# nlaha/genomics-rs

Measured on NVIDIA B200. Metric: GCUPS (affine NW/SW, score+traceback), higher is better.
Workload: dtype int32

## Files before the change

### genomics_rs_b200/_lib.py

```python
from __future__ import annotations

import ctypes as C
import os
import threading

_HERE = os.path.dirname(os.path.abspath(__file__))
LIB_PATH = os.environ.get("GX_LIB_PATH") or os.path.join(_HERE, "libgxalign.so")

GX_OK = 0
GX_FLAG_TRACEBACK = 1
GX_FLAG_LCS_AT_MAX = 2
GX_FLAG_START_CELL = 4

EXPORTS = [
    "gx_init", "gx_shutdown", "gx_device_count", "gx_strerror", "gx_last_error", "gx_version", "gx_check_scores",
    "gx_align_pair", "gx_align_batch", "gx_score_batch", "gx_plan_create", "gx_plan_upload", "gx_plan_execute",
    "gx_plan_fetch", "gx_plan_fetch_scores", "gx_plan_destroy", "gx_plan_stat", "gx_plan_debug_timeline", "gx_replay_ops", "gx_k0_measure",
    "gx_band_range", "gx_band_create", "gx_band_export", "gx_band_connect", "gx_band_upload", "gx_band_execute",
    "gx_band_score", "gx_band_stat", "gx_band_destroy", "gx_nw_score_banded", "gx_debug_planes", "gx_debug_tile_order",
]


class GxScores(C.Structure):
    _fields_ = [("s_match", C.c_int32), ("s_mismatch", C.c_int32), ("g", C.c_int32), ("h", C.c_int32)]


class GxResult(C.Structure):
    _fields_ = [
        ("score", C.c_int64),
        ("start_i", C.c_uint64), ("start_j", C.c_uint64), ("end_i", C.c_uint64), ("end_j", C.c_uint64),
        ("n_ops", C.c_uint64), ("matches", C.c_uint64), ("mismatches", C.c_uint64),
        ("gap_extensions", C.c_uint64), ("opening_gaps", C.c_uint64), ("lcs_at_first_max", C.c_uint64),
        ("fill_ms", C.c_double), ("walk_ms", C.c_double),
    ]


class GxError(RuntimeError):
    def __init__(self, status: int, detail: str = ""):
        self.status = status
        super().__init__(f"libgxalign status {status}: {detail}")


_lib = None
_lock = threading.Lock()
_inited_device = None


def load() -> C.CDLL:
    global _lib
    if _lib is not None:
        return _lib
    with _lock:
        if _lib is not None:
            return _lib
        if not os.path.exists(LIB_PATH):
            raise ImportError(
                f"{LIB_PATH} is missing: build it with `python -m genomics_rs_b200.build` "
                "(nvcc, sm_100a).  genomics_rs_b200 has no CPU or PyTorch fallback.")
        lib = C.CDLL(LIB_PATH)
        vp, u64, i32 = C.c_void_p, C.c_uint64, C.c_int
        lib.gx_init.argtypes = [i32]; lib.gx_init.restype = i32
        lib.gx_shutdown.argtypes = []; lib.gx_shutdown.restype = None
        lib.gx_device_count.argtypes = []; lib.gx_device_count.restype = i32
        lib.gx_strerror.argtypes = [i32]; lib.gx_strerror.restype = C.c_char_p
        lib.gx_last_error.argtypes = []; lib.gx_last_error.restype = C.c_char_p
        lib.gx_version.argtypes = []; lib.gx_version.restype = C.c_char_p
        lib.gx_check_scores.argtypes = [GxScores, u64, u64]; lib.gx_check_scores.restype = i32
        lib.gx_align_pair.argtypes = [vp, u64, vp, u64, GxScores, i32, i32, C.POINTER(GxResult), vp, u64]
        lib.gx_align_pair.restype = i32
        lib.gx_align_batch.argtypes = [vp, u64, vp, vp, vp, vp, u64, GxScores, i32, i32, vp, vp, vp]
        lib.gx_align_batch.restype = i32
        lib.gx_score_batch.argtypes = [vp, u64, vp, vp, vp, vp, u64, GxScores, i32, vp]
        lib.gx_score_batch.restype = i32
        lib.gx_plan_create.argtypes = [vp, vp, u64, GxScores, i32, i32, C.POINTER(vp)]; lib.gx_plan_create.restype = i32
        lib.gx_plan_upload.argtypes = [vp, vp, u64, vp, vp]; lib.gx_plan_upload.restype = i32
        lib.gx_plan_execute.argtypes = [vp]; lib.gx_plan_execute.restype = i32
        lib.gx_plan_fetch.argtypes = [vp, vp, vp, vp]; lib.gx_plan_fetch.restype = i32
        lib.gx_plan_fetch_scores.argtypes = [vp, vp]; lib.gx_plan_fetch_scores.restype = i32
        lib.gx_plan_destroy.argtypes = [vp]; lib.gx_plan_destroy.restype = None
        lib.gx_plan_stat.argtypes = [vp, i32]; lib.gx_plan_stat.restype = C.c_double
        lib.gx_plan_debug_timeline.argtypes = [vp, vp, u64]; lib.gx_plan_debug_timeline.restype = i32
        lib.gx_replay_ops.argtypes = [vp, u64, u64, u64, vp, vp]; lib.gx_replay_ops.restype = i32
        lib.gx_k0_measure.argtypes = [vp, i32]; lib.gx_k0_measure.restype = i32
        lib.gx_band_range.argtypes = [u64, i32, i32, C.POINTER(u64), C.POINTER(u64)]; lib.gx_band_range.restype = i32
        lib.gx_band_create.argtypes = [u64, u64, i32, i32, i32, GxScores, C.POINTER(vp)]; lib.gx_band_create.restype = i32
        lib.gx_band_export.argtypes = [vp, vp, u64]; lib.gx_band_export.restype = i32
        lib.gx_band_connect.argtypes = [vp, vp, vp]; lib.gx_band_connect.restype = i32
        lib.gx_band_upload.argtypes = [vp, vp, vp]; lib.gx_band_upload.restype = i32
        lib.gx_band_execute.argtypes = [vp]; lib.gx_band_execute.restype = i32
        lib.gx_band_score.argtypes = [vp, C.POINTER(C.c_int64), C.POINTER(i32)]; lib.gx_band_score.restype = i32
        lib.gx_band_stat.argtypes = [vp, i32]; lib.gx_band_stat.restype = C.c_double
        lib.gx_band_destroy.argtypes = [vp]; lib.gx_band_destroy.restype = None
        lib.gx_nw_score_banded.argtypes = [vp, u64, vp, u64, GxScores, i32, C.POINTER(C.c_int64)]
        lib.gx_nw_score_banded.restype = i32
        lib.gx_debug_tile_order.argtypes = [vp, vp, u64, i32, i32, vp, u64, C.POINTER(u64)]; lib.gx_debug_tile_order.restype = i32
        lib.gx_debug_planes.argtypes = [vp, u64, vp, u64, GxScores, i32, vp, vp, vp]; lib.gx_debug_planes.restype = i32
        _lib = lib
    return _lib


def check(status: int) -> None:
    if status != GX_OK:
        lib = load()
        detail = lib.gx_strerror(status).decode()
        extra = lib.gx_last_error().decode()
        raise GxError(status, f"{detail}{' -- ' + extra if extra else ''}")


def ensure_init(device: int | None = None) -> C.CDLL:
    global _inited_device
    lib = load()
    if _inited_device is None:
        if device is None:
            device = int(os.environ.get("LOCAL_RANK", "0"))
        check(lib.gx_init(device))
        _inited_device = device
    return lib


def shutdown() -> None:
    global _inited_device
    if _lib is not None and _inited_device is not None:
        _lib.gx_shutdown()
        _inited_device = None
```

### genomics_rs_b200/csrc/gx_api.cu

```cuda
#include <algorithm>
#include <cstdio>
#include <cstdlib>
#include <cstring>
#include <mutex>
#include <new>
#include <string>
#include <thread>
#include <vector>

#include "../../include/gxalign.h"
#include "gx_fill.cuh"
#include "gx_lcs.cuh"
#include "gx_reads.cuh"
#include "gx_walk.cuh"

namespace gx {

static_assert(sizeof(DevResult) == sizeof(gx_result), "DevResult must mirror gx_result");
static_assert(sizeof(PairDesc) == 104, "PairDesc layout");
static_assert(warp_smem_bytes(2) % 16 == 0 && warp_smem_bytes(4) % 16 == 0 && warp_smem_bytes(8) % 16 == 0 && warp_smem_bytes(16) % 16 == 0,
              "per-warp smem must keep 16 B alignment");

struct Block {
    void *ptr;
    size_t size;
    bool free;
};

struct Ctx {
    int device = -1;
    int sm_count = 0;
    cudaStream_t stream = nullptr;
    cudaEvent_t ev[4] = {nullptr, nullptr, nullptr, nullptr};
    std::vector<Block> pool;
    static constexpr int NLANES = 3;
    cudaStream_t lane_stream[NLANES] = {nullptr, nullptr, nullptr};
    cudaEvent_t lane_done[NLANES] = {nullptr, nullptr, nullptr};
    int *lane_scores_host[NLANES] = {nullptr, nullptr, nullptr};
    uint4 *lane_rec_host[NLANES] = {nullptr, nullptr, nullptr};
    size_t lane_scores_cap = 0;
    int host_threads = 1;
    uint8_t *ops_stage = nullptr;
    size_t ops_stage_cap = 0;
    std::string last_error;
    size_t pool_bytes = 0;
};

static Ctx *g_ctx = nullptr;
static std::recursive_mutex g_mu;
static thread_local std::string g_err;

static int fail_cuda(cudaError_t e, const char *what) {
    char buf[512];
    snprintf(buf, sizeof buf, "%s: %s (%s)", what, cudaGetErrorString(e), cudaGetErrorName(e));
    g_err = buf;
    if (g_ctx) g_ctx->last_error = buf;
    return GX_ERR_CUDA;
}
#define GX_GUARD_END                                                  \
    catch (const std::bad_alloc &) {                                  \
        g_err = "host allocation failed";                             \
        return GX_ERR_NOMEM;                                          \
    }                                                                 \
    catch (...) {                                                     \
        g_err = "unexpected C++ exception inside libgxalign";         \
        return GX_ERR_INTERNAL;                                       \
    }
#define CK(call)                                        \
    do {                                                \
        cudaError_t e__ = (call);                       \
        if (e__ != cudaSuccess) return fail_cuda(e__, #call); \
    } while (0)

static int pool_alloc(Ctx *c, size_t bytes, void **out) {
    if (bytes == 0) bytes = 16;
    bytes = (bytes + 511) & ~size_t(511);
    int best = -1;
    for (size_t k = 0; k < c->pool.size(); ++k) {
        Block &b = c->pool[k];
        if (b.free && b.size >= bytes && b.size <= 2 * bytes + (1u << 20))
            if (best < 0 || b.size < c->pool[best].size) best = (int)k;
    }
    if (best >= 0) {
        c->pool[best].free = false;
        *out = c->pool[best].ptr;
        return GX_OK;
    }
    void *p = nullptr;
    cudaError_t e = cudaMalloc(&p, bytes);
    if (e != cudaSuccess) {
        for (auto it = c->pool.begin(); it != c->pool.end();) {
            if (it->free) {
                cudaFree(it->ptr);
                c->pool_bytes -= it->size;
                it = c->pool.erase(it);
            } else ++it;
        }
        cudaGetLastError();
        e = cudaMalloc(&p, bytes);
        if (e != cudaSuccess) {
            cudaGetLastError();
            g_err = "device allocation of " + std::to_string(bytes) + " bytes failed";
            return GX_ERR_NOMEM;
        }
    }
    c->pool.push_back({p, bytes, false});
    c->pool_bytes += bytes;
    *out = p;
    return GX_OK;
}
static void pool_free(Ctx *c, void *p) {
    if (!p) return;
    for (auto &b : c->pool)
        if (b.ptr == p) {
            b.free = true;
            return;
        }
}

struct Tunables {
    int r = -1, batch = -1, code_band = -1, band_resident = 1;
    int k = -1, chain1 = -1, tickets = -1, resident = -1, wpc = -1, grid_cap = -1, pad_keys = 0, poll_nap = 0, start_lead = 0,
        fill_stats = 0, walk_stats = 0, walk_rows = 0, no_stream = 0, reads32 = 0, test_abort = 0;
};
static int env_int(const char *name, int dflt) {
    const char *e = getenv(name);
    return e ? atoi(e) : dflt;
}
static Tunables read_tunables() {
    Tunables t;
    t.k = env_int("GX_K", -1);
    t.r = env_int("GX_R", -1);
    t.batch = env_int("GX_BATCH", -1);
    t.band_resident = env_int("GX_BAND_RESIDENT", 1);
    t.code_band = env_int("GX_CODE_BAND", -1);
    t.chain1 = env_int("GX_CHAIN1", -1);
    t.tickets = getenv("GX_TICKETS") ? 1 : -1;
    t.resident = env_int("GX_RESIDENT", -1);
    t.wpc = env_int("GX_WPC", -1);
    t.grid_cap = env_int("GX_GRID_CAP", -1);
    t.pad_keys = getenv("GX_PAD_KEYS") ? 1 : 0;
    t.poll_nap = env_int("GX_POLL_NAP", 0);
    t.start_lead = env_int("GX_START_LEAD", 0);
    t.fill_stats = env_int("GX_FILL_STATS", 0);
    t.walk_stats = getenv("GX_WALK_STATS") ? 1 : 0;
    t.walk_rows = env_int("GX_WALK_ROWS", 0);
    t.no_stream = getenv("GX_NO_STREAM") ? 1 : 0;
    t.reads32 = getenv("GX_READS32") ? 1 : 0;
    t.test_abort = getenv("GX_TEST_ABORT") ? 1 : 0;
    return t;
}

enum PlanKind { KIND_WAVEFRONT = 0, KIND_READS = 1 };
typedef void (*FillKernel)(const FillParams);

}

struct gx_band;
struct gx_plan {
    gx::Ctx *ctx = nullptr;
    int kind = gx::KIND_WAVEFRONT;
    uint64_t n_pairs = 0;
    gx_scores sc{};
    gx::Tunables tun;
    int is_local = 0, flags = 0;
    int K = 8, R = 1;
    uint32_t cpb = 1;
    bool chain1 = false;
    int track = 0;
    bool traceback = false;
    std::vector<gx::PairDesc> pairs;
    std::vector<uint64_t> len1, len2;
    uint64_t n_tiles = 0;
    uint64_t n_strips = 0;
    uint64_t cells = 0;
    uint64_t code_bytes = 0, ops_bytes = 0, colbuf_entries = 0, top_entries = 0, progress_entries = 0, best_entries = 0;
    uint64_t blob_cap = 0;
    uint64_t max_len = 0;
    uint8_t *d_blob = nullptr;
    uint8_t *d_blob_sym = nullptr;
    uint8_t *d_lut = nullptr;
    unsigned long long *d_stats = nullptr;
    unsigned long long h_stats[8] = {0};
    unsigned long long *d_timeline = nullptr;
    bool prof = false;
    gx::PairDesc *d_pairs = nullptr;
    gx::TileDesc *d_tiles = nullptr;
    gx::TileDesc *d_strips = nullptr;
    bool resident = false;
    uint32_t pmax = 0;
    uint32_t *d_ctrl = nullptr;
    unsigned long long *d_colbuf = nullptr;
    int2 *d_top = nullptr;
    uint8_t *d_codes = nullptr;
    int4 *d_best = nullptr;
    bool lcs = false;
    int4 *d_first = nullptr;
    uint32_t *d_masks = nullptr, *d_carry = nullptr;
    uint32_t carry_words = 0;
    float lcs_ms = 0;
    gx::DevResult *d_results = nullptr;
    uint8_t *d_ops = nullptr;
    uint64_t *d_off1 = nullptr, *d_off2 = nullptr;
    uint32_t *d_len1 = nullptr, *d_len2 = nullptr;
    int *d_scores = nullptr;
    uint32_t parity = 0;
    bool uploaded = false, executed = false, colbuf_dirty = true;
    float fill_ms = 0, walk_ms = 0;
    int launches = 0;
    int retries = 0;
    int reads_bits = 0;
    bool code_band = false;
    uint8_t *d_tile_codes = nullptr;
    int band_fallbacks = 0;
    uint32_t left_band = 0;
    double code_cell_frac = 1.0;
    uint64_t h2d_bytes = 0, d2h_bytes = 0, dev_bytes = 0;
    gx_band *band = nullptr;
};

struct gx_band {
    gx_plan *plan = nullptr;
    uint64_t m = 0, n_total = 0;
    gx_scores sc{};
    int n_bands = 0, first = 0, last = 0;
    std::vector<uint64_t> col0, width;
    uint8_t *link = nullptr;
    std::vector<unsigned long long *> internal;
    void *left_base = nullptr, *right_base = nullptr;
    uint32_t epoch = 0;
    bool connected = false, poisoned = false, trivial = false;
    float fill_ms = 0;
};

namespace gx {

#define GX_COMBOS(X) X(4, 1) X(8, 1) X(16, 1)

#define GX_DECL(K, R)                                                  \
    FillKernel pick_fill_##K##_##R##_0(bool prof, bool L, bool C, int track); \
    FillKernel pick_fill_##K##_##R##_1(bool prof, bool L, bool C, int track);
GX_COMBOS(GX_DECL)
#undef GX_DECL

static bool combo_ok(int K, int R) {
#define GX_CHK(k, r) if (K == k && R == r) return true;
    GX_COMBOS(GX_CHK)
#undef GX_CHK
    return false;
}

static FillKernel pick_fill(int K, int R, bool prof, bool chain1, bool L, bool C, int track) {
#define GX_PICK(k, r) if (K == k && R == r) return chain1 ? pick_fill_##k##_##r##_1(prof, L, C, track) : pick_fill_##k##_##r##_0(prof, L, C, track);
    GX_COMBOS(GX_PICK)
#undef GX_PICK
    return nullptr;
}

static int launch_fill(gx_plan *pl, const FillParams &fp, int grid_cap, int track_override = -1) {
    Ctx *c = pl->ctx;
    const int K = pl->K;
    const bool L = pl->is_local != 0, C = pl->traceback;
    const bool banded = pl->code_band && track_override < 0 && C && !L;
    FillKernel kern = (track_override >= 0) ? pick_fill(K, pl->R, pl->prof, pl->chain1, L, false, track_override)
                      : banded              ? pick_fill(K, pl->R, pl->prof, pl->chain1, false, true, 4)
                                            : pick_fill(K, pl->R, pl->prof, pl->chain1, L, C, pl->track);
    if (!kern) {
        g_err = "no fill kernel for this (K, R)";
        return GX_ERR_INTERNAL;
    }
    int wpc = (pl->n_strips * 2 >= (uint64_t)c->sm_count * warps_per_sm(K)) ? WARPS_PER_CTA : 1;
    if (pl->tun.wpc >= 0) wpc = pl->tun.wpc == 1 ? 1 : WARPS_PER_CTA;
    if (pl->resident) wpc = 1;
    const size_t smem = (size_t)wpc * warp_smem_bytes(K);
    CK(cudaFuncSetAttribute(kern, cudaFuncAttributeMaxDynamicSharedMemorySize, (int)(WARPS_PER_CTA * warp_smem_bytes(K))));
    int occ = 0;
    CK(cudaOccupancyMaxActiveBlocksPerMultiprocessor(&occ, kern, wpc * 32, smem));
    if (occ < 1) occ = 1;
    const bool codes_kernel = C && track_override < 0;
    occ = std::min(occ, (codes_kernel ? warps_per_sm(K) : GX_SCORE_CTAS * WARPS_PER_CTA) / wpc);
    uint64_t cap = (uint64_t)c->sm_count * occ;
    FillParams fq = fp;
    fq.tile_codes = banded ? pl->d_tile_codes : nullptr;
    if (pl->resident && pl->n_strips > cap) {
        g_err = "resident-strips plan does not fit the device (fewer than 16 single-warp CTAs per SM)";
        return GX_ERR_INTERNAL;
    }
    if (pl->resident) {
        fq.pmax = pl->pmax;
        fq.tiles = pl->d_strips;
        fq.n_tiles = (uint32_t)(pl->n_strips * pl->pmax);
    }
    uint64_t want = fq.pmax ? pl->n_strips : (pl->n_tiles + wpc - 1) / wpc;
    if (pl->tun.grid_cap >= 0) grid_cap = pl->tun.grid_cap;
    if (grid_cap > 0 && (uint64_t)grid_cap < cap) cap = grid_cap;
    int grid = (int)std::min<uint64_t>(want, cap);
    if (grid < 1) grid = 1;
    if (pl->resident) {
        void *kargs[] = {(void *)&fq};
        CK(cudaLaunchCooperativeKernel((const void *)kern, dim3((unsigned)grid), dim3((unsigned)(wpc * 32)), kargs, smem, c->stream));
    } else {
        kern<<<grid, wpc * 32, smem, c->stream>>>(fq);
    }
    CK(cudaGetLastError());
    return GX_OK;
}

typedef void (*WalkKernel)(const WalkParams);
static int launch_walk(gx_plan *pl, WalkParams wp) {
    WalkKernel kern = nullptr;
#define GX_WALK(k, r) \
    if (pl->K == k && pl->R == r) kern = gx_walk_kernel<k, r>;
    GX_COMBOS(GX_WALK)
#undef GX_WALK
    if (!kern) {
        g_err = "no walk kernel for this (K, R)";
        return GX_ERR_INTERNAL;
    }
    const uint32_t row_cap = (uint32_t)std::max<uint64_t>(64, std::min<uint64_t>(512, (pl->max_len + 63) / 64 * 64));
    uint32_t rows = 0;
    for (uint32_t cand : {512u, 384u, 256u, 192u, 128u, 64u}) {
        if (cand > 256u && pl->K > 8) continue;
        const uint32_t r_ = std::min(cand, row_cap);
        const uint32_t per_sm = std::min<uint32_t>(2048u / WALK_THREADS, (227u * 1024u) / (walk_smem_bytes(pl->K, pl->R, r_) + 1024u));
        if (pl->n_pairs <= (uint64_t)per_sm * (uint64_t)pl->ctx->sm_count) {
            rows = r_;
            break;
        }
    }
    if (!rows) rows = pl->max_len <= 256 ? 64u : 128u;
    if (pl->tun.walk_rows >= 64 && pl->tun.walk_rows <= 512 && pl->tun.walk_rows % 64 == 0) rows = (uint32_t)pl->tun.walk_rows;
    wp.win_rows = rows;
    const uint32_t smem = wp.traceback ? walk_smem_bytes(pl->K, pl->R, rows) : 0u;
    CK(cudaFuncSetAttribute(kern, cudaFuncAttributeMaxDynamicSharedMemorySize, (int)walk_smem_bytes(pl->K, pl->R, 512u)));
    kern<<<(unsigned)pl->n_pairs, wp.traceback ? WALK_THREADS : 32, smem, pl->ctx->stream>>>(wp);
    CK(cudaGetLastError());
    return GX_OK;
}

static int check_scores_impl(gx_scores sc, uint64_t m, uint64_t n, bool local) {
    if (!(sc.h <= 0 && sc.g < 0 && (long long)sc.h + sc.g < 0)) return GX_ERR_SCORES;
    long long mx = std::max({std::llabs((long long)sc.s_match), std::llabs((long long)sc.s_mismatch), std::llabs((long long)sc.g)});
    long long lim = 1ll << 29;
    if (m > (1ull << 28) || n > (1ull << 28)) return GX_ERR_RANGE;
    if ((long long)(m + n + 2) * mx + std::llabs((long long)sc.h) >= lim) return GX_ERR_RANGE;
    if (local) {
        long long vmax = (long long)std::min(m, n) * std::max<long long>(sc.s_match, 0);
        if (vmax >= (1ll << 26)) return GX_ERR_RANGE;
    }
    return GX_OK;
}

static void plan_release(gx_plan *pl) {
    Ctx *c = pl->ctx;
    void *ptrs[] = {pl->d_tile_codes, pl->d_blob, pl->d_blob_sym, pl->d_lut, pl->d_stats, pl->d_timeline, pl->d_pairs, pl->d_tiles, pl->d_strips, pl->d_ctrl, pl->d_colbuf, pl->d_top, pl->d_codes, pl->d_best, pl->d_first, pl->d_masks, pl->d_carry,
                    pl->d_results, pl->d_ops, pl->d_off1, pl->d_off2, pl->d_len1, pl->d_len2, pl->d_scores};
    for (void *p : ptrs) pool_free(c, p);
}

}

using namespace gx;

extern "C" {

const char *gx_version(void) {
#ifdef GX_CHECKED
    return "gxalign 0.2 (sm_100a, checked build: device-side bounds assertions)";
#else
    return "gxalign 0.2 (sm_100a)";
#endif
}

const char *gx_strerror(int s) {
    switch (s) {
        case GX_OK: return "ok";
        case GX_ERR_ARG: return "invalid argument";
        case GX_ERR_SCORES: return "scores violate h <= 0, g < 0, h+g < 0";
        case GX_ERR_RANGE: return "sequence lengths x scores exceed the int32 cell range";
        case GX_ERR_OPS_CAP: return "ops buffer too small";
        case GX_ERR_NO_DEVICE: return "no sm_100 CUDA device (there is no CPU path)";
        case GX_ERR_CUDA: return "CUDA error";
        case GX_ERR_NOMEM: return "out of memory";
        case GX_ERR_NOT_INIT: return "gx_init not called";
        case GX_ERR_UNSUPPORTED: return "unsupported flag or mode";
        case GX_ERR_INTERNAL: return "internal error";
        default: return "unknown status";
    }
}

const char *gx_last_error(void) { return g_err.c_str(); }

int gx_device_count(void) {
    int n = 0;
    if (cudaGetDeviceCount(&n) != cudaSuccess) {
        cudaGetLastError();
        return 0;
    }
    int ok = 0;
    for (int d = 0; d < n; ++d) {
        int major = 0;
        if (cudaDeviceGetAttribute(&major, cudaDevAttrComputeCapabilityMajor, d) == cudaSuccess && major == 10) ok++;
    }
    return ok;
}

int gx_init(int device) try {
    std::lock_guard<std::recursive_mutex> lk(g_mu);
    int n = 0;
    if (cudaGetDeviceCount(&n) != cudaSuccess || n == 0) {
        cudaGetLastError();
        g_err = "no CUDA device visible";
        return GX_ERR_NO_DEVICE;
    }
    if (device < 0) {
        if (cudaGetDevice(&device) != cudaSuccess) return GX_ERR_NO_DEVICE;
    }
    if (device >= n) return GX_ERR_ARG;
    int major = 0;
    CK(cudaDeviceGetAttribute(&major, cudaDevAttrComputeCapabilityMajor, device));
    if (major != 10) {
        g_err = "device is not compute capability 10.x; libgxalign carries sm_100a code only";
        return GX_ERR_NO_DEVICE;
    }
    if (g_ctx && g_ctx->device == device) return GX_OK;
    if (g_ctx) return GX_ERR_ARG;
    CK(cudaSetDevice(device));
    Ctx *c = new (std::nothrow) Ctx();
    if (!c) return GX_ERR_NOMEM;
    c->device = device;
    CK(cudaDeviceGetAttribute(&c->sm_count, cudaDevAttrMultiProcessorCount, device));
    CK(cudaStreamCreateWithFlags(&c->stream, cudaStreamNonBlocking));
    for (auto &e : c->ev) CK(cudaEventCreate(&e));
    for (int k = 0; k < Ctx::NLANES; ++k) {
        CK(cudaStreamCreateWithFlags(&c->lane_stream[k], cudaStreamNonBlocking));
        CK(cudaEventCreateWithFlags(&c->lane_done[k], cudaEventDisableTiming));
    }
    {
        int ndev = 1;
        cudaGetDeviceCount(&ndev);
        const unsigned hw = std::thread::hardware_concurrency();
        c->host_threads = (int)std::max(1u, std::min(8u, hw / (unsigned)std::max(1, ndev)));
        if (const char *e = getenv("GX_HOST_THREADS")) c->host_threads = std::max(1, atoi(e));
    }
    g_ctx = c;
    return GX_OK;
}
GX_GUARD_END

static void band_cache_drop();
static void plan_cache_drop();

void gx_shutdown(void) {
    std::lock_guard<std::recursive_mutex> lk(g_mu);
    if (!g_ctx) return;
    cudaSetDevice(g_ctx->device);
    cudaStreamSynchronize(g_ctx->stream);
    band_cache_drop();
    plan_cache_drop();
    for (auto &b : g_ctx->pool) cudaFree(b.ptr);
    for (auto &e : g_ctx->ev) cudaEventDestroy(e);
    for (int k = 0; k < Ctx::NLANES; ++k) {
        if (g_ctx->lane_stream[k]) cudaStreamDestroy(g_ctx->lane_stream[k]);
        if (g_ctx->lane_done[k]) cudaEventDestroy(g_ctx->lane_done[k]);
        if (g_ctx->lane_scores_host[k]) cudaFreeHost(g_ctx->lane_scores_host[k]);
        if (g_ctx->lane_rec_host[k]) cudaFreeHost(g_ctx->lane_rec_host[k]);
    }
    if (g_ctx->ops_stage) cudaFreeHost(g_ctx->ops_stage);
    cudaStreamDestroy(g_ctx->stream);
    delete g_ctx;
    g_ctx = nullptr;
}

int gx_check_scores(gx_scores sc, uint64_t m, uint64_t n) { return check_scores_impl(sc, m, n, true); }

int gx_replay_ops(const uint8_t *ops, uint64_t n_ops, uint64_t start_i, uint64_t start_j, uint32_t *ops_i, uint32_t *ops_j) {
    if ((!ops && n_ops) || !ops_i || !ops_j) return GX_ERR_ARG;
    uint64_t i = start_i, j = start_j;
    for (uint64_t k = 0; k < n_ops; ++k) {
        ops_i[k] = (uint32_t)i;
        ops_j[k] = (uint32_t)j;
        switch (ops[k]) {
            case GX_MATCH:
            case GX_MISMATCH:
                i = i ? i - 1 : 0;
                j = j ? j - 1 : 0;
                break;
            case GX_INSERT:
            case GX_OPEN_INSERT: j = j ? j - 1 : 0; break;
            case GX_DELETE:
            case GX_OPEN_DELETE: i = i ? i - 1 : 0; break;
            default: return GX_ERR_ARG;
        }
    }
    return GX_OK;
}

}


static void build_ticket_order(const std::vector<uint32_t> &S, const std::vector<uint32_t> &P, const std::vector<uint64_t> &sbase,
                               std::vector<TileDesc> &tiles) {
    const size_t n_pairs = S.size();
    constexpr uint64_t TS = PANEL_H / 64;
    uint64_t vmax = 0;
    std::vector<uint32_t> live;
    for (size_t q = 0; q < n_pairs; ++q)
        if (S[q] && P[q]) {
            vmax = std::max<uint64_t>(vmax, (uint64_t)(P[q] - 1) * TS + sbase[q] + S[q] - 1);
            live.push_back((uint32_t)q);
        }
    for (uint64_t v = 0; v <= vmax && !live.empty(); ++v) {
        size_t keep = 0;
        for (size_t li = 0; li < live.size(); ++li) {
            const uint32_t q = live[li];
            const uint64_t last = (uint64_t)(P[q] - 1) * TS + sbase[q] + S[q] - 1;
            if (v <= last) live[keep++] = q;
            if (v < sbase[q]) continue;
            const uint64_t sv = v - sbase[q];
            const uint64_t p_hi = std::min<uint64_t>(P[q] - 1, sv / TS);
            const uint64_t p_lo = (sv >= S[q]) ? (sv - S[q] + 1 + TS - 1) / TS : 0;
            for (uint64_t p2 = p_lo; p2 <= p_hi; ++p2) tiles.push_back({q, (uint32_t)p2, (uint32_t)(sv - TS * p2), 0});
        }
        live.resize(keep);
    }
}

static int plan_create_locked(const uint64_t *len1, const uint64_t *len2, uint64_t n_pairs, gx_scores sc, int is_local, int flags,
                              const uint64_t *band_col0, gx_plan **out) {
    if (!out) return GX_ERR_ARG;
    *out = nullptr;
    if (!g_ctx) return GX_ERR_NOT_INIT;
    if ((!len1 || !len2) && n_pairs) return GX_ERR_ARG;
    if (n_pairs >= (1ull << 31)) return GX_ERR_RANGE;
    Ctx *c = g_ctx;
    CK(cudaSetDevice(c->device));
    uint64_t max_len = 0;
    for (uint64_t q = 0; q < n_pairs; ++q) {
        int rc = check_scores_impl(sc, len1[q], len2[q], is_local != 0);
        if (rc) return rc;
        max_len = std::max({max_len, len1[q], len2[q]});
    }
    if (n_pairs == 0) {
        int rc = check_scores_impl(sc, 0, 0, is_local != 0);
        if (rc) return rc;
    }
    gx_plan *pl = new (std::nothrow) gx_plan();
    if (!pl) return GX_ERR_NOMEM;
    pl->ctx = c;
    pl->n_pairs = n_pairs;
    pl->sc = sc;
    pl->tun = read_tunables();
    pl->is_local = is_local ? 1 : 0;
    pl->flags = flags;
    pl->traceback = (flags & GX_FLAG_TRACEBACK) != 0;
    pl->track = is_local ? ((pl->traceback || (flags & GX_FLAG_START_CELL)) ? 2 : 1) : 0;
    pl->len1.assign(len1, len1 + n_pairs);
    pl->len2.assign(len2, len2 + n_pairs);
    pl->max_len = max_len;
    for (uint64_t q = 0; q < n_pairs; ++q) pl->cells += (len1[q] + 1) * (len2[q] + 1);

    pl->lcs = (flags & GX_FLAG_LCS_AT_MAX) != 0 && !band_col0;
    if (pl->lcs) {
        long long mx = std::max({std::llabs((long long)sc.s_match), std::llabs((long long)sc.s_mismatch), std::llabs((long long)sc.g)});
        if (n_pairs > 65536 || (long long)(2 * max_len + 2) * mx + std::llabs((long long)sc.h) >= (1ll << 26)) {
            delete pl;
            return n_pairs > 65536 ? GX_ERR_UNSUPPORTED : GX_ERR_RANGE;
        }
    }
    const bool reads = !pl->lcs && !band_col0 && !pl->traceback && pl->track != 2 && n_pairs >= 1024 && max_len <= (uint64_t)READS_MAX_LEN &&
                       (!is_local || sc.s_mismatch < 0);
    pl->kind = reads ? KIND_READS : KIND_WAVEFRONT;
    int rc = GX_OK;
    auto A = [&](size_t bytes, void **p) {
        if (rc == GX_OK) {
            rc = pool_alloc(c, bytes, p);
            if (rc == GX_OK) pl->dev_bytes += (bytes + 511) & ~size_t(511);
        }
    };
    if (pl->kind == KIND_READS) {
        A(n_pairs * 8, (void **)&pl->d_off1);
        A(n_pairs * 8, (void **)&pl->d_off2);
        A(n_pairs * 4, (void **)&pl->d_len1);
        A(n_pairs * 4, (void **)&pl->d_len2);
        A(n_pairs * 4, (void **)&pl->d_scores);
        if (rc == GX_OK) {
            std::vector<uint32_t> l1(n_pairs), l2(n_pairs);
            for (uint64_t q = 0; q < n_pairs; ++q) {
                l1[q] = (uint32_t)len1[q];
                l2[q] = (uint32_t)len2[q];
            }
            cudaError_t e = cudaMemcpyAsync(pl->d_len1, l1.data(), n_pairs * 4, cudaMemcpyHostToDevice, c->stream);
            if (e == cudaSuccess) e = cudaMemcpyAsync(pl->d_len2, l2.data(), n_pairs * 4, cudaMemcpyHostToDevice, c->stream);
            if (e == cudaSuccess) e = cudaStreamSynchronize(c->stream);
            if (e != cudaSuccess) rc = fail_cuda(e, "upload lengths");
        }
        if (rc != GX_OK) {
            plan_release(pl);
            delete pl;
            return rc;
        }
        *out = pl;
        return GX_OK;
    }

    {
        const uint64_t resident = (uint64_t)c->sm_count * warps_per_sm(16);
        uint64_t strips16 = 0, strips8 = 0;
        for (uint64_t q = 0; q < n_pairs; ++q)
            if (len1[q] && len2[q]) {
                strips16 += (len2[q] + 511) / 512;
                strips8 += (len2[q] + 255) / 256;
            }
        (void)strips16;
        pl->K = (strips8 * 10 >= resident * 12 || max_len < 2048) ? 8 : 4;
        if (combo_ok(pl->tun.k, 1)) pl->K = pl->tun.k;
        pl->R = 1;
        if (pl->tun.r > 0 && combo_ok(pl->K, pl->tun.r)) pl->R = pl->tun.r;
        {
            uint64_t strips = 0;
            for (uint64_t q = 0; q < n_pairs; ++q)
                if (len1[q] && len2[q]) strips += (len2[q] + 32 * pl->K - 1) / (32 * pl->K);
            pl->chain1 = strips * 4 < resident;
            pl->n_strips = strips;
        }
        if (pl->tun.chain1 >= 0) pl->chain1 = pl->tun.chain1 != 0;
        const int kb = pl->K == 16 ? 4 : pl->K == 8 ? 3 : 2;
        if (pl->track == 2 && pl->chain1 && -((long long)sc.h + sc.g) >= (1ll << (31 - kb))) pl->chain1 = false;
    }
    const int K = pl->K, R = pl->R, W = 32 * K;
    {
        const uint64_t ns = pl->n_strips;
        pl->resident = ns > 0 && ns * 10 <= (uint64_t)c->sm_count * warps_per_sm(K) * 7 && pl->tun.tickets < 0;
        if (pl->tun.resident >= 0 && ns <= (uint64_t)c->sm_count * warps_per_sm(K)) pl->resident = pl->tun.resident != 0;
    }
    const uint32_t SPC = 64u / (uint32_t)(R * K), CPB_MAX = std::max(1u, 32u / (SPC * (uint32_t)R));
    {
        uint32_t steps = 32u;
        if (pl->tun.batch > 0) steps = (uint32_t)pl->tun.batch;
        uint32_t cpb = std::max(1u, steps / SPC);
        while (cpb & (cpb - 1)) cpb &= cpb - 1;
        pl->cpb = std::min(cpb, CPB_MAX);
    }
    const uint32_t CPB = pl->cpb, BATCH = CPB * SPC;
    pl->pairs.resize(n_pairs);
    std::vector<TileDesc> tiles;
    std::vector<uint64_t> sbase(n_pairs, 0);
    uint64_t n_tiles_total = 0;
    uint64_t colbuf = 0, top = 0, codes = 0, ops = 0, progress = 0, best = 0;
    uint64_t strip_base = 0;
    for (uint64_t q = 0; q < n_pairs; ++q) {
        PairDesc &pd = pl->pairs[q];
        memset(&pd, 0, sizeof pd);
        const uint64_t m = len1[q], n = len2[q];
        pd.m = (uint32_t)m;
        pd.n = (uint32_t)n;
        const bool interior = m > 0 && n > 0;
        pd.S = interior ? (uint32_t)((n + W - 1) / W) : 0;
        pd.P = interior ? (uint32_t)((m + PANEL_H - 1) / PANEL_H) : 0;
        pd.colbuf_off = colbuf;
        pd.top_off = top;
        pd.codes_off = codes;
        pd.ops_off = ops;
        pd.progress_off = (uint32_t)progress;
        pd.tile_base = (uint32_t)best;
        const uint32_t rows_max = (uint32_t)std::min<uint64_t>(m, PANEL_H);
        pd.tile_code_bytes = interior ? tile_batches(rows_max, (uint32_t)R, BATCH) * CPB * 32 * 16 : 0;
        pd.col0 = band_col0 ? (uint32_t)band_col0[q] : 0u;
        if (interior) {
            colbuf += (uint64_t)(pd.S - 1) * m;
            top += n;
            progress += pd.S;
            if (progress >= (1ull << 32) || best + (uint64_t)pd.S * pd.P >= (1ull << 32)) {
                delete pl;
                return GX_ERR_RANGE;
            }
            best += (uint64_t)pd.S * pd.P;
            if (pl->traceback) codes += (uint64_t)pd.S * pd.P * pd.tile_code_bytes;
        }
        if (pl->traceback) ops += ((m + n + 1) + 31) & ~uint64_t(31);
        sbase[q] = strip_base;
        n_tiles_total += (uint64_t)pd.S * pd.P;
        if (band_col0) strip_base += pd.S;
    }
    if (n_tiles_total >= (1ull << 32) - 65536) {
        delete pl;
        return GX_ERR_RANGE;
    }
    if (!pl->resident) {
        std::vector<uint32_t> Sv(n_pairs), Pv(n_pairs);
        for (uint64_t q = 0; q < n_pairs; ++q) {
            Sv[q] = pl->pairs[q].S;
            Pv[q] = pl->pairs[q].P;
        }
        tiles.reserve(n_tiles_total);
        build_ticket_order(Sv, Pv, sbase, tiles);
    }
    pl->n_tiles = n_tiles_total;
    std::vector<TileDesc> strips;
    {
        if (pl->resident) {
            for (uint64_t q = 0; q < n_pairs; ++q) pl->pmax = std::max(pl->pmax, pl->pairs[q].P);
            for (uint64_t q = 0; q < n_pairs; ++q)
                for (uint32_t s2 = 0; s2 < pl->pairs[q].S; ++s2)
                    for (uint32_t p2 = 0; p2 < pl->pmax; ++p2)
                        strips.push_back(p2 < pl->pairs[q].P ? TileDesc{(uint32_t)q, p2, s2, 0u} : TileDesc{0xffffffffu, 0u, 0u, 0u});
        }
    }
    pl->code_bytes = codes;
    pl->ops_bytes = ops;
    pl->colbuf_entries = colbuf;
    pl->top_entries = top;
    pl->progress_entries = progress;
    pl->best_entries = best;

    A(n_pairs * sizeof(PairDesc), (void **)&pl->d_pairs);
    A(tiles.size() * sizeof(TileDesc), (void **)&pl->d_tiles);
    if (pl->resident) A(strips.size() * sizeof(TileDesc), (void **)&pl->d_strips);
    A((16 + progress) * 4, (void **)&pl->d_ctrl);
    A(colbuf * 8, (void **)&pl->d_colbuf);
    A(top * 8, (void **)&pl->d_top);
    if (pl->traceback) A(codes, (void **)&pl->d_codes);
    if (pl->is_local) A(best * 16, (void **)&pl->d_best);
    if (pl->lcs) {
        pl->carry_words = (uint32_t)((max_len + 31) / 32 + 1);
        A(best * 16 + 16, (void **)&pl->d_first);
        A((size_t)n_pairs * 256 * LCS_BLOCK_WORDS * 4, (void **)&pl->d_masks);
        A((size_t)n_pairs * 2 * pl->carry_words * 4 + 16, (void **)&pl->d_carry);
    }
    A(n_pairs * sizeof(DevResult), (void **)&pl->d_results);
    std::vector<uint8_t> tile_codes;
    if (pl->traceback && !is_local && !band_col0 && (!pl->resident || pl->tun.band_resident != 0) && pl->tun.code_band != 0 && best > 0) {
        tile_codes.assign(best, 1);
        double with = 0, all = 0;
        for (uint64_t q = 0; q < n_pairs; ++q) {
            const PairDesc &pd = pl->pairs[q];
            const uint64_t dmn = pd.m > pd.n ? pd.m - pd.n : pd.n - pd.m;
            const uint64_t cw = pl->tun.code_band > 0 ? (uint64_t)pl->tun.code_band : 1024 + dmn;
            for (uint32_t p2 = 0; p2 < pd.P; ++p2) {
                const double rows = (double)std::min<uint64_t>(PANEL_H, pd.m - (uint64_t)p2 * PANEL_H);
                for (uint32_t s2 = 0; s2 < pd.S; ++s2) {
                    const double cols = (double)std::min<uint64_t>((uint64_t)W, pd.n - (uint64_t)s2 * W);
                    const bool in = tile_in_code_band(pd.m, pd.n, p2, s2, (uint32_t)W, cw);
                    tile_codes[pd.tile_base + (uint64_t)p2 * pd.S + s2] = in ? 1 : 0;
                    all += rows * cols;
                    if (in) with += rows * cols;
                }
            }
        }
        pl->code_cell_frac = all > 0 ? with / all : 1.0;
        pl->code_band = pl->code_cell_frac < 0.9;
        if (!pl->code_band) pl->code_cell_frac = 1.0;
        if (pl->code_band) A(best, (void **)&pl->d_tile_codes);
    }
    if (pl->traceback) A(ops, (void **)&pl->d_ops);
    if (rc == GX_OK && pl->code_band) {
        cudaError_t e = cudaMemcpyAsync(pl->d_tile_codes, tile_codes.data(), best, cudaMemcpyHostToDevice, c->stream);
        if (e == cudaSuccess) e = cudaStreamSynchronize(c->stream);
        if (e != cudaSuccess) rc = fail_cuda(e, "upload tile code flags");
    }
    if (rc == GX_OK && (!tiles.empty() || !strips.empty())) {
        cudaError_t e = cudaSuccess;
        if (!tiles.empty()) e = cudaMemcpyAsync(pl->d_tiles, tiles.data(), tiles.size() * sizeof(TileDesc), cudaMemcpyHostToDevice, c->stream);
        if (e == cudaSuccess && pl->resident)
            e = cudaMemcpyAsync(pl->d_strips, strips.data(), strips.size() * sizeof(TileDesc), cudaMemcpyHostToDevice, c->stream);
        if (e == cudaSuccess) e = cudaStreamSynchronize(c->stream);
        if (e != cudaSuccess) rc = fail_cuda(e, "upload tiles");
    }
    if (rc != GX_OK) {
        plan_release(pl);
        delete pl;
        return rc;
    }
    *out = pl;
    return GX_OK;
}


template <class F>
static void host_parallel(int threads, uint64_t n, F &&f) {
    if (threads <= 1 || n < (1u << 15)) {
        f(0, (uint64_t)0, n);
        return;
    }
    std::vector<std::thread> th;
    th.reserve(threads - 1);
    const uint64_t per = (n + threads - 1) / threads;
    for (int t = 1; t < threads; ++t) {
        const uint64_t lo = std::min<uint64_t>(n, per * t), hi = std::min<uint64_t>(n, per * (t + 1));
        th.emplace_back([&f, t, lo, hi] { f(t, lo, hi); });
    }
    f(0, (uint64_t)0, std::min<uint64_t>(n, per));
    for (auto &t : th) t.join();
}

static int score_batch_streamed(const uint8_t *blob, uint64_t blob_len, const uint64_t *off1, const uint64_t *len1,
                                const uint64_t *off2, const uint64_t *len2, uint64_t n_pairs, gx_scores sc, int is_local,
                                int64_t *scores, bool force32) {
    std::lock_guard<std::recursive_mutex> lk(g_mu);
    if (!g_ctx) return GX_ERR_NOT_INIT;
    Ctx *c = g_ctx;
    if (n_pairs < (1u << 18) || (is_local && sc.s_mismatch >= 0)) return GX_ERR_UNSUPPORTED;
    int rc = check_scores_impl(sc, READS_MAX_LEN, READS_MAX_LEN, is_local != 0);
    if (rc) return rc;
    CK(cudaSetDevice(c->device));
    constexpr int NL = Ctx::NLANES;
    const uint64_t CH = 1u << 18;
    const int T = std::min(c->host_threads, 16);
    if (c->lane_scores_cap < CH) {
        for (int k = 0; k < NL; ++k) {
            if (c->lane_scores_host[k]) cudaFreeHost(c->lane_scores_host[k]);
            c->lane_scores_host[k] = nullptr;
            if (c->lane_rec_host[k]) cudaFreeHost(c->lane_rec_host[k]);
            c->lane_rec_host[k] = nullptr;
            if (cudaHostAlloc((void **)&c->lane_scores_host[k], CH * sizeof(int), cudaHostAllocDefault) != cudaSuccess ||
                cudaHostAlloc((void **)&c->lane_rec_host[k], CH * sizeof(uint4), cudaHostAllocDefault) != cudaSuccess) {
                cudaGetLastError();
                c->lane_scores_cap = 0;
                return GX_ERR_NOMEM;
            }
        }
        c->lane_scores_cap = CH;
    }
    struct Lane {
        uint8_t *blob = nullptr;
        size_t blob_cap = 0;
        uint4 *rec = nullptr;
        int *scores = nullptr;
        uint64_t first = 0, count = 0;
        bool busy = false;
    } lane[NL];
    auto release = [&]() {
        for (auto &L : lane) {
            void *ptrs[] = {L.blob, L.rec, L.scores};
            for (void *p : ptrs) pool_free(c, p);
        }
    };
    auto drain = [&](int k) -> int {
        Lane &L = lane[k];
        if (!L.busy) return GX_OK;
        cudaError_t e = cudaEventSynchronize(c->lane_done[k]);
        if (e != cudaSuccess) return fail_cuda(e, "cudaEventSynchronize(lane_done)");
        const int *src = c->lane_scores_host[k];
        int64_t *dst = scores + L.first;
        for (uint64_t q = 0; q < L.count; ++q) dst[q] = src[q];
        L.busy = false;
        return GX_OK;
    };
    for (int k = 0; k < NL && rc == GX_OK; ++k) {
        Lane &L = lane[k];
        rc = pool_alloc(c, CH * sizeof(uint4), (void **)&L.rec);
        if (!rc) rc = pool_alloc(c, CH * 4, (void **)&L.scores);
    }
    struct Part {
        uint64_t lo = UINT64_MAX, hi = 0, maxlen = 0, sum = 0, bad = 0;
    };
    std::vector<Part> parts((size_t)std::max(T, 1));
#define CKB(call)                                   \
    {                                               \
        cudaError_t e__ = (call);                   \
        if (e__ != cudaSuccess) {                   \
            rc = fail_cuda(e__, #call);             \
            break;                                  \
        }                                           \
    }
    for (uint64_t first = 0, ci = 0; first < n_pairs && rc == GX_OK; first += CH, ++ci) {
        const int k = (int)(ci % NL);
        Lane &L = lane[k];
        const uint64_t count = std::min<uint64_t>(CH, n_pairs - first);
        const uint64_t *o1 = off1 + first, *o2 = off2 + first, *l1 = len1 + first, *l2 = len2 + first;
        for (auto &p : parts) p = Part();
        host_parallel(T, count, [&](int tid, uint64_t a, uint64_t b) {
            Part p;
            for (uint64_t q = a; q < b; ++q) {
                const uint64_t a0 = o1[q], a1 = a0 + l1[q], b0 = o2[q], b1 = b0 + l2[q];
                p.bad |= (uint64_t)(a1 > blob_len) | (uint64_t)(b1 > blob_len) | (uint64_t)(a1 < a0) | (uint64_t)(b1 < b0);
                p.lo = std::min(p.lo, std::min(a0, b0));
                p.hi = std::max(p.hi, std::max(a1, b1));
                p.maxlen = std::max(p.maxlen, std::max(l1[q], l2[q]));
                p.sum += l1[q] + l2[q];
            }
            parts[(size_t)tid] = p;
        });
        uint64_t lo = UINT64_MAX, hi = 0, maxlen = 0, sum = 0, badbits = 0;
        for (const auto &p : parts) {
            lo = std::min(lo, p.lo);
            hi = std::max(hi, p.hi);
            maxlen = std::max(maxlen, p.maxlen);
            sum += p.sum;
            badbits |= p.bad;
        }
        if (badbits) {
            rc = GX_ERR_ARG;
            break;
        }
        if (maxlen > (uint64_t)READS_MAX_LEN || hi - lo > 4 * sum + (1u << 20) || hi - lo >= (1ull << 32)) {
            rc = GX_ERR_UNSUPPORTED;
            break;
        }
        rc = drain(k);
        if (rc) break;
        const uint64_t span = hi > lo ? hi - lo : 0;
        if (L.blob_cap < span + 64) {
            pool_free(c, L.blob);
            L.blob = nullptr;
            L.blob_cap = 0;
            rc = pool_alloc(c, span + span / 4 + 64, (void **)&L.blob);
            if (rc) break;
            L.blob_cap = span + span / 4 + 64;
        }
        cudaStream_t st = c->lane_stream[k];
        if (span) CKB(cudaMemcpyAsync(L.blob, blob + lo, span, cudaMemcpyHostToDevice, st));
        {
            uint4 *rec = c->lane_rec_host[k];
            host_parallel(T, count, [&](int, uint64_t a, uint64_t b) {
                for (uint64_t q = a; q < b; ++q)
                    rec[q] = make_uint4((uint32_t)(o1[q] - lo), (uint32_t)(o2[q] - lo), (uint32_t)l1[q], (uint32_t)l2[q]);
            });
        }
        CKB(cudaMemcpyAsync(L.rec, c->lane_rec_host[k], count * sizeof(uint4), cudaMemcpyHostToDevice, st));
        ReadsParams rp;
        rp.blob = L.blob;
        rp.off1 = rp.off2 = nullptr;
        rp.len1 = rp.len2 = nullptr;
        rp.rec = L.rec;
        rp.n_pairs = (uint32_t)count;
        rp.scores = L.scores;
        rp.results = nullptr;
        rp.a = sc.s_match;
        rp.b = sc.s_mismatch;
        rp.g = sc.g;
        rp.h = sc.h;
        rp.is_local = is_local ? 1 : 0;
        if (launch_reads(rp, (int)maxlen, c->sm_count, st, force32) != 0) {
            rc = GX_ERR_UNSUPPORTED;
            break;
        }
        CKB(cudaGetLastError());
        CKB(cudaMemcpyAsync(c->lane_scores_host[k], L.scores, count * 4, cudaMemcpyDeviceToHost, st));
        CKB(cudaEventRecord(c->lane_done[k], st));
        L.first = first;
        L.count = count;
        L.busy = true;
    }
#undef CKB
    for (int k = 0; k < NL && rc == GX_OK; ++k) rc = drain(k);
    if (rc != GX_OK) {
        for (int k = 0; k < NL; ++k) cudaStreamSynchronize(c->lane_stream[k]);
        cudaGetLastError();
    }
    release();
    return rc;
}

extern "C" {

int gx_plan_create(const uint64_t *len1, const uint64_t *len2, uint64_t n_pairs, gx_scores sc, int is_local, int flags,
                   gx_plan **out) try {
    std::lock_guard<std::recursive_mutex> lk(g_mu);
    return plan_create_locked(len1, len2, n_pairs, sc, is_local, flags, nullptr, out);
}
GX_GUARD_END

int gx_plan_upload(gx_plan *pl, const uint8_t *blob, uint64_t blob_len, const uint64_t *off1, const uint64_t *off2) try {
    std::lock_guard<std::recursive_mutex> lk(g_mu);
    if (!pl || (!blob && blob_len) || ((!off1 || !off2) && pl->n_pairs)) return GX_ERR_ARG;
    Ctx *c = pl->ctx;
    CK(cudaSetDevice(c->device));
    for (uint64_t q = 0; q < pl->n_pairs; ++q)
        if (off1[q] > blob_len || pl->len1[q] > blob_len - off1[q] || off2[q] > blob_len || pl->len2[q] > blob_len - off2[q])
            return GX_ERR_ARG;
    if (!pl->d_blob || pl->blob_cap < blob_len + 64) {
        pool_free(c, pl->d_blob);
        pl->d_blob = nullptr;
        int rc = pool_alloc(c, blob_len + 64, (void **)&pl->d_blob);
        if (rc) return rc;
        pl->blob_cap = blob_len + 64;
        pl->dev_bytes += blob_len + 64;
    }
    if (blob_len) CK(cudaMemcpyAsync(pl->d_blob, blob, blob_len, cudaMemcpyHostToDevice, c->stream));
    CK(cudaMemsetAsync(pl->d_blob + blob_len, 0, 64, c->stream));
    pl->h2d_bytes = blob_len;
    if (pl->kind == KIND_READS) {
        if (pl->n_pairs) {
            CK(cudaMemcpyAsync(pl->d_off1, off1, pl->n_pairs * 8, cudaMemcpyHostToDevice, c->stream));
            CK(cudaMemcpyAsync(pl->d_off2, off2, pl->n_pairs * 8, cudaMemcpyHostToDevice, c->stream));
            pl->h2d_bytes += pl->n_pairs * 16;
        }
    } else {
        bool seen[256] = {false};
        int nsym = 0;
        uint8_t lut[256];
        memset(lut, 255, sizeof lut);
        {
            std::vector<std::pair<uint64_t, uint64_t>> segs;
            segs.reserve(2 * pl->n_pairs);
            for (uint64_t q = 0; q < pl->n_pairs; ++q) {
                segs.push_back({off1[q], pl->len1[q]});
                segs.push_back({off2[q], pl->len2[q]});
            }
            std::sort(segs.begin(), segs.end());
            segs.erase(std::unique(segs.begin(), segs.end()), segs.end());
            uint64_t done_to = 0;
            for (size_t k = 0; k < segs.size() && nsym <= 4; ++k) {
                uint64_t lo = std::max(segs[k].first, done_to), hi = segs[k].first + segs[k].second;
                for (uint64_t x = lo; x < hi; ++x) {
                    const uint8_t ch = blob[x];
                    if (!seen[ch]) {
                        seen[ch] = true;
                        if (nsym < 4) lut[ch] = (uint8_t)(8 * nsym);
                        nsym++;
                    }
                }
                done_to = std::max(done_to, hi);
            }
        }
        {
            const long long hg = (long long)pl->sc.h + pl->sc.g;
            const long long v[4] = {pl->sc.s_match - hg, pl->sc.s_mismatch - hg, pl->sc.s_match, pl->sc.s_mismatch};
            bool fits = true;
            for (long long x : v) fits = fits && x >= -128 && x <= 127;
            pl->prof = nsym <= 4 && fits && pl->n_tiles > 0;
        }
        if (pl->prof) {
            for (int x = 0; x < 256; ++x)
                if (lut[x] == 255) lut[x] = 0;
            if (!pl->d_lut) {
                int rc = pool_alloc(c, 256, (void **)&pl->d_lut);
                if (rc) return rc;
            }
            pool_free(c, pl->d_blob_sym);
            pl->d_blob_sym = nullptr;
            int rc = pool_alloc(c, blob_len + 64, (void **)&pl->d_blob_sym);
            if (rc) return rc;
            pl->dev_bytes += blob_len + 64;
            CK(cudaMemcpyAsync(pl->d_lut, lut, 256, cudaMemcpyHostToDevice, c->stream));
            const int grid = (int)std::min<uint64_t>((blob_len + 64 + 255) / 256, (uint64_t)c->sm_count * 8);
            gx_encode_kernel<<<grid, 256, 0, c->stream>>>(pl->d_blob, pl->d_blob_sym, (size_t)blob_len + 64, pl->d_lut);
            CK(cudaGetLastError());
        }
        for (uint64_t q = 0; q < pl->n_pairs; ++q) {
            pl->pairs[q].s1_off = off1[q];
            pl->pairs[q].s2_off = off2[q];
        }
        if (pl->n_pairs) {
            CK(cudaMemcpyAsync(pl->d_pairs, pl->pairs.data(), pl->n_pairs * sizeof(PairDesc), cudaMemcpyHostToDevice, c->stream));
            pl->h2d_bytes += pl->n_pairs * sizeof(PairDesc);
        }
    }
    CK(cudaStreamSynchronize(c->stream));
    pl->uploaded = true;
    return GX_OK;
}
GX_GUARD_END

static int plan_execute_once(gx_plan *pl, bool *aborted);

static int plan_build_tickets(gx_plan *pl) {
    Ctx *c = pl->ctx;
    const size_t np = pl->pairs.size();
    std::vector<uint32_t> Sv(np), Pv(np);
    std::vector<uint64_t> sbase(np, 0);
    uint64_t base = 0;
    for (size_t q = 0; q < np; ++q) {
        Sv[q] = pl->pairs[q].S;
        Pv[q] = pl->pairs[q].P;
        sbase[q] = base;
        if (pl->band) base += Sv[q];
    }
    std::vector<TileDesc> tiles;
    tiles.reserve(pl->n_tiles);
    build_ticket_order(Sv, Pv, sbase, tiles);
    if (tiles.size() != pl->n_tiles) return GX_ERR_INTERNAL;
    if (tiles.empty()) return GX_OK;
    pool_free(c, pl->d_tiles);
    pl->d_tiles = nullptr;
    int rc = pool_alloc(c, tiles.size() * sizeof(TileDesc), (void **)&pl->d_tiles);
    if (rc) return rc;
    CK(cudaMemcpyAsync(pl->d_tiles, tiles.data(), tiles.size() * sizeof(TileDesc), cudaMemcpyHostToDevice, c->stream));
    CK(cudaStreamSynchronize(c->stream));
    return GX_OK;
}

int gx_plan_execute(gx_plan *pl) try {
    std::lock_guard<std::recursive_mutex> lk(g_mu);
    if (!pl) return GX_ERR_ARG;
    if (!pl->uploaded) return GX_ERR_ARG;
    bool aborted = false;
    int rc = plan_execute_once(pl, &aborted);
    if (rc == GX_ERR_INTERNAL && aborted && pl->resident && !(pl->band && pl->band->n_bands > pl->band->last - pl->band->first)) {
        pl->resident = false;
        pl->retries++;
        int rb = plan_build_tickets(pl);
        if (rb) return rb;
        pl->colbuf_dirty = true;
        rc = plan_execute_once(pl, &aborted);
    }
    if (rc == GX_OK && pl->code_band && pl->left_band != 0) {
        const float f0 = pl->fill_ms, w0 = pl->walk_ms;
        const int l0 = pl->launches;
        pl->code_band = false;
        pl->code_cell_frac = 1.0;
        pl->band_fallbacks++;
        rc = plan_execute_once(pl, &aborted);
        pl->fill_ms += f0;
        pl->walk_ms += w0;
        pl->launches += l0;
    }
    return rc;
}
GX_GUARD_END

static int plan_execute_once(gx_plan *pl, bool *aborted) {
    Ctx *c = pl->ctx;
    CK(cudaSetDevice(c->device));
    pl->launches = 0;
    pl->fill_ms = pl->walk_ms = 0;
    const gx_scores sc = pl->sc;
    if (pl->n_pairs == 0) {
        pl->executed = true;
        return GX_OK;
    }
    if (pl->kind == KIND_READS) {
        ReadsParams rp;
        rp.blob = pl->d_blob;
        rp.off1 = pl->d_off1;
        rp.off2 = pl->d_off2;
        rp.len1 = pl->d_len1;
        rp.len2 = pl->d_len2;
        rp.rec = nullptr;
        rp.n_pairs = (uint32_t)pl->n_pairs;
        rp.scores = pl->d_scores;
        rp.results = nullptr;
        rp.a = sc.s_match;
        rp.b = sc.s_mismatch;
        rp.g = sc.g;
        rp.h = sc.h;
        rp.is_local = pl->is_local;
        CK(cudaEventRecord(c->ev[0], c->stream));
        int rc = launch_reads(rp, (int)pl->max_len, c->sm_count, c->stream, pl->tun.reads32 != 0, &pl->reads_bits);
        if (rc == -1) return GX_ERR_UNSUPPORTED;
        CK(cudaGetLastError());
        CK(cudaEventRecord(c->ev[1], c->stream));
        CK(cudaStreamSynchronize(c->stream));
        CK(cudaEventElapsedTime(&pl->fill_ms, c->ev[0], c->ev[1]));
        pl->launches = 1;
        pl->executed = true;
        return GX_OK;
    }

    gx_band *bd = pl->band;
    if (bd && bd->poisoned) {
        g_err = "band plan is unusable after a failed execute (neighbouring bands are out of step): create it again";
        return GX_ERR_INTERNAL;
    }
    CK(cudaEventRecord(c->ev[0], c->stream));
    if (pl->colbuf_dirty) {
        if (pl->colbuf_entries) CK(cudaMemsetAsync(pl->d_colbuf, 0xff, pl->colbuf_entries * 8, c->stream));
        if (bd) {
            if (bd->epoch != 0 && bd->n_bands > bd->last - bd->first) {
                bd->poisoned = true;
                return GX_ERR_INTERNAL;
            }
            for (auto *lk : bd->internal) CK(cudaMemsetAsync(lk, 0xff, bd->m * 8, c->stream));
        }
        pl->parity = 0;
    }
    pl->colbuf_dirty = true;
    CK(cudaMemsetAsync(pl->d_ctrl, 0, (16 + pl->progress_entries) * 4, c->stream));
    FillParams fp;
    fp.blob = pl->d_blob;
    fp.blob_sym = pl->prof ? pl->d_blob_sym : nullptr;
    fp.one = 1u;
    fp.stats = nullptr;
    fp.timeline = nullptr;
    fp.pad_keys = (sc.s_mismatch >= 0 || pl->tun.pad_keys) ? 1u : 0u;
    fp.poll_nap = (uint32_t)pl->tun.poll_nap;
    fp.start_lead = (uint32_t)pl->tun.start_lead;
    if (pl->tun.fill_stats) {
        if (!pl->d_stats) {
            int rc = pool_alloc(c, 64, (void **)&pl->d_stats);
            if (rc) return rc;
        }
        CK(cudaMemsetAsync(pl->d_stats, 0, 64, c->stream));
        fp.stats = pl->d_stats;
        if (pl->tun.fill_stats >= 2) {
            if (!pl->d_timeline) {
                int rc = pool_alloc(c, (std::max<uint64_t>(pl->n_tiles, pl->n_strips * pl->pmax) + 1) * 32, (void **)&pl->d_timeline);
                if (rc) return rc;
            }
            fp.timeline = pl->d_timeline;
        }
    }
    fp.pairs = pl->d_pairs;
    fp.n_pairs = (uint32_t)pl->n_pairs;
    fp.code_bytes = pl->code_bytes;
    fp.tiles = pl->d_tiles;
    fp.n_tiles = (uint32_t)pl->n_tiles;
    fp.pmax = 0;
    fp.parity = pl->parity;
    fp.cpb = pl->cpb;
    fp.epoch = bd ? bd->epoch + 1 : 0;
    fp.ticket = pl->d_ctrl;
    fp.progress = pl->d_ctrl + 16;
    fp.colbuf = pl->d_colbuf;
    fp.top = pl->d_top;
    fp.codes = pl->d_codes;
    fp.tile_best = pl->d_best;
    fp.g = sc.g;
    fp.h = sc.h;
    fp.hg = sc.h + sc.g;
    fp.ap = sc.s_match - fp.hg;
    fp.bp = sc.s_mismatch - fp.hg;
    if (pl->n_tiles) {
        int rc = launch_fill(pl, fp, 0);
        if (rc) return rc;
        pl->launches++;
    }
    CK(cudaEventRecord(c->ev[1], c->stream));
    if (bd && bd->left_base) {
        gx_band_ack_kernel<<<1, 1, 0, c->stream>>>(reinterpret_cast<uint32_t *>(bd->left_base), bd->epoch + 1);
        CK(cudaGetLastError());
        pl->launches++;
    }
    WalkParams wp;
    wp.blob = pl->d_blob;
    wp.pairs = pl->d_pairs;
    wp.n_pairs = (uint32_t)pl->n_pairs;
    wp.top = pl->d_top;
    wp.codes = pl->d_codes;
    wp.tile_best = pl->d_best;
    wp.results = pl->d_results;
    wp.ops = pl->d_ops;
    wp.g = sc.g;
    wp.h = sc.h;
    wp.hg = fp.hg;
    wp.kcols_log2 = pl->K == 16 ? 4 : pl->K == 4 ? 2 : 3;
    wp.is_local = pl->is_local;
    wp.traceback = pl->traceback ? 1 : 0;
    wp.have_best = pl->track == 2 ? 1 : 0;
    wp.debug = pl->tun.walk_stats;
    wp.check = pl->d_ctrl + 2;
    wp.left_band = pl->d_ctrl + 3;
    wp.tile_codes = pl->code_band ? pl->d_tile_codes : nullptr;
    wp.code_bytes = pl->code_bytes;
    wp.ops_bytes = pl->ops_bytes;
    {
        int rc = launch_walk(pl, wp);
        if (rc) return rc;
        pl->launches++;
    }
    CK(cudaEventRecord(c->ev[2], c->stream));
    uint32_t ctrl_words[3] = {0, 0, 0};
    CK(cudaMemcpyAsync(ctrl_words, pl->d_ctrl + 1, 12, cudaMemcpyDeviceToHost, c->stream));
    uint32_t ctrl2[2] = {0, 0};
    if (pl->lcs) {
        if (pl->n_tiles) {
            CK(cudaMemsetAsync(pl->d_ctrl, 0, (16 + pl->progress_entries) * 4, c->stream));
            FillParams fq = fp;
            fq.parity = pl->parity ^ 1u;
            fq.codes = nullptr;
            fq.tile_best = pl->d_first;
            fq.stats = nullptr;
            fq.timeline = nullptr;
            int rc = launch_fill(pl, fq, 0, 3);
            if (rc) return rc;
            pl->launches++;
            CK(cudaMemcpyAsync(ctrl2, pl->d_ctrl + 1, 8, cudaMemcpyDeviceToHost, c->stream));
        }
        LcsParams lp;
        lp.blob = pl->d_blob;
        lp.pairs = pl->d_pairs;
        lp.n_pairs = (uint32_t)pl->n_pairs;
        lp.tile_first = pl->d_first;
        lp.masks = pl->d_masks;
        lp.carry = pl->d_carry;
        lp.carry_words = pl->carry_words;
        lp.results = pl->d_results;
        gx_lcs_kernel<<<(unsigned)pl->n_pairs, 32, 0, c->stream>>>(lp);
        CK(cudaGetLastError());
        pl->launches++;
        CK(cudaEventRecord(c->ev[3], c->stream));
    }
    if (fp.stats) CK(cudaMemcpyAsync(pl->h_stats, pl->d_stats, 64, cudaMemcpyDeviceToHost, c->stream));
    CK(cudaStreamSynchronize(c->stream));
    uint32_t abort_word = ctrl_words[0];
    const uint32_t abort_word2 = ctrl2[0];
    if (ctrl_words[1] || ctrl2[1]) {
        g_err = "checked build: device bounds check failed at site " + std::to_string(ctrl_words[1] ? ctrl_words[1] : ctrl2[1]);
        return GX_ERR_INTERNAL;
    }
    if (pl->tun.test_abort && pl->resident && pl->retries == 0) abort_word = 1;
    if (abort_word || abort_word2) {
        g_err = "fill kernel aborted: a tile waited > SPIN_LIMIT polls for a dependency";
        if (bd && bd->n_bands > bd->last - bd->first) bd->poisoned = true;
        *aborted = true;
        return GX_ERR_INTERNAL;
    }
    if (bd) bd->epoch++;
    pl->left_band = ctrl_words[2];
    CK(cudaEventElapsedTime(&pl->fill_ms, c->ev[0], c->ev[1]));
    CK(cudaEventElapsedTime(&pl->walk_ms, c->ev[1], c->ev[2]));
    if (pl->lcs) CK(cudaEventElapsedTime(&pl->lcs_ms, c->ev[2], c->ev[3]));
    if (!(pl->lcs && pl->n_tiles)) pl->parity ^= 1u;
    pl->colbuf_dirty = false;
    pl->executed = true;
    return GX_OK;
}

int gx_plan_fetch(gx_plan *pl, gx_result *out, uint8_t *ops_blob, const uint64_t *ops_off) try {
    std::lock_guard<std::recursive_mutex> lk(g_mu);
    if (!pl || (!out && pl->n_pairs)) return GX_ERR_ARG;
    if (!pl->executed) return GX_ERR_ARG;
    if (pl->traceback && pl->n_pairs && (!ops_blob || !ops_off)) return GX_ERR_ARG;
    Ctx *c = pl->ctx;
    CK(cudaSetDevice(c->device));
    if (pl->n_pairs == 0) return GX_OK;
    if (pl->kind == KIND_READS) {
        std::vector<int> sc32(pl->n_pairs);
        CK(cudaMemcpyAsync(sc32.data(), pl->d_scores, pl->n_pairs * 4, cudaMemcpyDeviceToHost, c->stream));
        CK(cudaStreamSynchronize(c->stream));
        pl->d2h_bytes = pl->n_pairs * 4;
        for (uint64_t q = 0; q < pl->n_pairs; ++q) {
            gx_result r;
            memset(&r, 0, sizeof r);
            r.score = sc32[q];
            r.start_i = r.end_i = pl->len1[q];
            r.start_j = r.end_j = pl->len2[q];
            r.fill_ms = pl->fill_ms;
            out[q] = r;
        }
        return GX_OK;
    }
    CK(cudaMemcpyAsync(out, pl->d_results, pl->n_pairs * sizeof(gx_result), cudaMemcpyDeviceToHost, c->stream));
    pl->d2h_bytes = pl->n_pairs * sizeof(gx_result);
    if (pl->traceback) {
        if (c->ops_stage_cap < pl->ops_bytes) {
            if (c->ops_stage) cudaFreeHost(c->ops_stage);
            c->ops_stage = nullptr;
            c->ops_stage_cap = 0;
            const size_t want = pl->ops_bytes + pl->ops_bytes / 4 + 4096;
            if (cudaHostAlloc((void **)&c->ops_stage, want, cudaHostAllocDefault) != cudaSuccess) {
                cudaGetLastError();
                return GX_ERR_NOMEM;
            }
            c->ops_stage_cap = want;
        }
        CK(cudaMemcpyAsync(c->ops_stage, pl->d_ops, pl->ops_bytes, cudaMemcpyDeviceToHost, c->stream));
        pl->d2h_bytes += pl->ops_bytes;
    }
    CK(cudaStreamSynchronize(c->stream));
    int rc = GX_OK;
    const bool walk_dbg = pl->tun.walk_stats != 0;
    for (uint64_t q = 0; q < pl->n_pairs; ++q) {
        if (!walk_dbg) out[q].fill_ms = pl->fill_ms;
        if (!walk_dbg) out[q].walk_ms = pl->walk_ms;
        if (pl->traceback) {
            const uint64_t cap = ops_off[q + 1] - ops_off[q];
            if (out[q].n_ops > cap) {
                rc = GX_ERR_OPS_CAP;
                continue;
            }
            memcpy(ops_blob + ops_off[q], c->ops_stage + pl->pairs[q].ops_off, out[q].n_ops);
        }
    }
    return rc;
}
GX_GUARD_END

int gx_plan_fetch_scores(gx_plan *pl, int64_t *scores) try {
    std::lock_guard<std::recursive_mutex> lk(g_mu);
    if (!pl || (!scores && pl->n_pairs)) return GX_ERR_ARG;
    if (!pl->executed) return GX_ERR_ARG;
    Ctx *c = pl->ctx;
    CK(cudaSetDevice(c->device));
    if (pl->n_pairs == 0) return GX_OK;
    if (pl->kind == KIND_READS) {
        std::vector<int> sc32(pl->n_pairs);
        CK(cudaMemcpyAsync(sc32.data(), pl->d_scores, pl->n_pairs * 4, cudaMemcpyDeviceToHost, c->stream));
        CK(cudaStreamSynchronize(c->stream));
        pl->d2h_bytes = pl->n_pairs * 4;
        for (uint64_t q = 0; q < pl->n_pairs; ++q) scores[q] = sc32[q];
        return GX_OK;
    }
    std::vector<gx_result> res(pl->n_pairs);
    CK(cudaMemcpyAsync(res.data(), pl->d_results, pl->n_pairs * sizeof(gx_result), cudaMemcpyDeviceToHost, c->stream));
    CK(cudaStreamSynchronize(c->stream));
    pl->d2h_bytes = pl->n_pairs * sizeof(gx_result);
    for (uint64_t q = 0; q < pl->n_pairs; ++q) scores[q] = res[q].score;
    return GX_OK;
}
GX_GUARD_END

int gx_plan_debug_timeline(gx_plan *pl, uint64_t *out, uint64_t cap_words) {
    std::lock_guard<std::recursive_mutex> lk(g_mu);
    if (!pl || !out || !pl->d_timeline || cap_words < pl->n_tiles * 4) return GX_ERR_ARG;
    CK(cudaSetDevice(pl->ctx->device));
    CK(cudaMemcpy(out, pl->d_timeline, pl->n_tiles * 32, cudaMemcpyDeviceToHost));
    return GX_OK;
}

int gx_debug_tile_order(const uint64_t *len1, const uint64_t *len2, uint64_t n_pairs, int K, int bands, uint32_t *out,
                        uint64_t cap_tiles, uint64_t *n_tiles) try {
    if ((!len1 || !len2) && n_pairs) return GX_ERR_ARG;
    if (!n_tiles || (K != 2 && K != 4 && K != 8 && K != 16)) return GX_ERR_ARG;
    std::vector<uint32_t> S(n_pairs), P(n_pairs);
    std::vector<uint64_t> sbase(n_pairs, 0);
    uint64_t base = 0, total = 0;
    for (uint64_t q = 0; q < n_pairs; ++q) {
        const bool interior = len1[q] > 0 && len2[q] > 0;
        S[q] = interior ? (uint32_t)((len2[q] + 32 * K - 1) / (32 * K)) : 0;
        P[q] = interior ? (uint32_t)((len1[q] + PANEL_H - 1) / PANEL_H) : 0;
        sbase[q] = base;
        if (bands) base += S[q];
        total += (uint64_t)S[q] * P[q];
    }
    *n_tiles = total;
    if (!out) return GX_OK;
    if (cap_tiles < total) return GX_ERR_ARG;
    std::vector<TileDesc> tiles;
    tiles.reserve(total);
    build_ticket_order(S, P, sbase, tiles);
    if (tiles.size() != total) return GX_ERR_INTERNAL;
    for (size_t k = 0; k < tiles.size(); ++k) {
        out[3 * k + 0] = tiles[k].pair;
        out[3 * k + 1] = tiles[k].p;
        out[3 * k + 2] = tiles[k].s;
    }
    return GX_OK;
}
GX_GUARD_END

double gx_plan_stat(const gx_plan *pl, int what) {
    if (!pl) return -1.0;
    switch (what) {
        case 0: return pl->fill_ms;
        case 1: return pl->walk_ms;
        case 2: return pl->launches;
        case 3: return (double)pl->cells;
        case 4: return (double)pl->code_bytes;
        case 5: return (double)pl->dev_bytes;
        case 6: return (double)pl->h2d_bytes;
        case 7: return (double)pl->d2h_bytes;
        case 8: return (double)pl->n_tiles;
        case 9: return (double)pl->kind;
        case 15: return (double)pl->K;
        case 19: return (double)pl->R;
        case 20: return (double)pl->retries;
        case 23: return pl->code_cell_frac;
        case 24: return (double)pl->band_fallbacks;
        case 22: return (double)(pl->cpb * (64u / (uint32_t)(pl->R * pl->K)));
        case 21: return pl->resident ? 1.0 : 0.0;
        case 17: return pl->chain1 ? 1.0 : 0.0;
        case 18: return pl->lcs_ms;
        case 25: return pl->prof ? 1.0 : 0.0;
        case 26: return (double)pl->reads_bits;
        case 10: case 11: case 12: case 13: case 14: return (double)pl->h_stats[what - 10];
        default: return -1.0;
    }
}

void gx_plan_destroy(gx_plan *pl) {
    std::lock_guard<std::recursive_mutex> lk(g_mu);
    if (!pl) return;
    plan_release(pl);
    delete pl;
}


int gx_band_range(uint64_t n_total, int n_bands, int band, uint64_t *col0, uint64_t *width) {
    if (n_bands < 1 || band < 0 || band >= n_bands || !col0 || !width) return GX_ERR_ARG;
    uint64_t lo, hi;
    if (n_total / (uint64_t)n_bands >= std::max<uint64_t>(4096, 512ull * n_bands)) {
        const uint64_t base = ((n_total + n_bands - 1) / n_bands + 511) / 512 * 512;
        lo = std::min<uint64_t>(n_total, base * band);
        hi = std::min<uint64_t>(n_total, base * (band + 1));
    } else {
        const uint64_t q = n_total / n_bands, r = n_total % n_bands;
        lo = q * band + std::min<uint64_t>(band, r);
        hi = lo + q + ((uint64_t)band < r ? 1 : 0);
    }
    *col0 = lo;
    *width = hi - lo;
    return GX_OK;
}

static void band_free(gx_band *b) {
    if (!b) return;
    if (b->plan) gx_plan_destroy(b->plan);
    if (g_ctx) {
        for (auto *p : b->internal) pool_free(g_ctx, p);
        if (b->left_base) cudaIpcCloseMemHandle(b->left_base);
        if (b->right_base) cudaIpcCloseMemHandle(b->right_base);
        if (b->link) cudaFree(b->link);
        cudaGetLastError();
    }
    delete b;
}

int gx_band_create(uint64_t m, uint64_t n_total, int n_bands, int first_band, int last_band, gx_scores sc, gx_band **out) try {
    std::lock_guard<std::recursive_mutex> lk(g_mu);
    if (!out) return GX_ERR_ARG;
    *out = nullptr;
    if (!g_ctx) return GX_ERR_NOT_INIT;
    if (n_bands < 1 || first_band < 0 || last_band <= first_band || last_band > n_bands) return GX_ERR_ARG;
    int rc = check_scores_impl(sc, m, n_total, false);
    if (rc) return rc;
    if (m > 0 && n_total > 0 && n_total < (uint64_t)n_bands) return GX_ERR_ARG;
    Ctx *c = g_ctx;
    CK(cudaSetDevice(c->device));
    gx_band *b = new (std::nothrow) gx_band();
    if (!b) return GX_ERR_NOMEM;
    b->m = m;
    b->n_total = n_total;
    b->sc = sc;
    b->n_bands = n_bands;
    b->first = first_band;
    b->last = last_band;
    b->trivial = (m == 0 || n_total == 0);
    if (b->trivial) {
        *out = b;
        return GX_OK;
    }
    const int nl = last_band - first_band;
    std::vector<uint64_t> l1(nl, m), l2(nl);
    b->col0.resize(nl);
    b->width.resize(nl);
    for (int q = 0; q < nl; ++q) {
        gx_band_range(n_total, n_bands, first_band + q, &b->col0[q], &b->width[q]);
        l2[q] = b->width[q];
        if (l2[q] == 0) {
            delete b;
            return GX_ERR_ARG;
        }
    }
    rc = plan_create_locked(l1.data(), l2.data(), (uint64_t)nl, sc, 0, 0, b->col0.data(), &b->plan);
    if (rc) {
        delete b;
        return rc;
    }
    b->plan->band = b;
    for (int q = 0; q + 1 < nl && rc == GX_OK; ++q) {
        unsigned long long *p = nullptr;
        rc = pool_alloc(c, m * 8, (void **)&p);
        if (rc == GX_OK) b->internal.push_back(p);
    }
    if (rc == GX_OK && nl < n_bands) {
        cudaError_t e = cudaMalloc((void **)&b->link, 256 + m * 8);
        if (e == cudaSuccess) e = cudaMemsetAsync(b->link, 0xff, 256 + m * 8, c->stream);
        if (e == cudaSuccess) e = cudaMemsetAsync(b->link, 0, 256, c->stream);
        if (e == cudaSuccess) e = cudaStreamSynchronize(c->stream);
        if (e != cudaSuccess) {
            cudaGetLastError();
            rc = (e == cudaErrorMemoryAllocation) ? GX_ERR_NOMEM : fail_cuda(e, "band link block");
        }
    }
    if (rc != GX_OK) {
        band_free(b);
        return rc;
    }
    for (int q = 0; q < nl; ++q) {
        PairDesc &pd = b->plan->pairs[q];
        pd.inbox = (q > 0) ? b->internal[q - 1] : nullptr;
        pd.outbox = (q + 1 < nl) ? b->internal[q] : nullptr;
        pd.ack = nullptr;
    }
    b->connected = (nl == n_bands);
    *out = b;
    return GX_OK;
}
GX_GUARD_END

int gx_band_export(gx_band *b, void *handle, uint64_t handle_cap) {
    std::lock_guard<std::recursive_mutex> lk(g_mu);
    if (!b || !handle || handle_cap < GX_BAND_HANDLE_BYTES) return GX_ERR_ARG;
    static_assert(sizeof(cudaIpcMemHandle_t) <= GX_BAND_HANDLE_BYTES, "handle size");
    memset(handle, 0, GX_BAND_HANDLE_BYTES);
    if (!b->link) return GX_OK;
    CK(cudaSetDevice(g_ctx->device));
    cudaIpcMemHandle_t h;
    CK(cudaIpcGetMemHandle(&h, b->link));
    memcpy(handle, &h, sizeof h);
    return GX_OK;
}

int gx_band_connect(gx_band *b, const void *left_handle, const void *right_handle) try {
    std::lock_guard<std::recursive_mutex> lk(g_mu);
    if (!b) return GX_ERR_ARG;
    if (b->trivial) return GX_OK;
    const bool need_left = b->first > 0, need_right = b->last < b->n_bands;
    if ((need_left && !left_handle) || (need_right && !right_handle)) return GX_ERR_ARG;
    if (b->connected) return GX_OK;
    CK(cudaSetDevice(g_ctx->device));
    const int nl = b->last - b->first;
    if (need_left) {
        cudaIpcMemHandle_t h;
        memcpy(&h, left_handle, sizeof h);
        CK(cudaIpcOpenMemHandle(&b->left_base, h, cudaIpcMemLazyEnablePeerAccess));
        b->plan->pairs[0].inbox = reinterpret_cast<const unsigned long long *>(b->link + 256);
    }
    if (need_right) {
        cudaIpcMemHandle_t h;
        memcpy(&h, right_handle, sizeof h);
        CK(cudaIpcOpenMemHandle(&b->right_base, h, cudaIpcMemLazyEnablePeerAccess));
        b->plan->pairs[nl - 1].outbox = reinterpret_cast<unsigned long long *>(static_cast<uint8_t *>(b->right_base) + 256);
        b->plan->pairs[nl - 1].ack = reinterpret_cast<const uint32_t *>(b->link);
    }
    b->connected = true;
    if (b->plan->uploaded) {
        CK(cudaMemcpyAsync(b->plan->d_pairs, b->plan->pairs.data(), nl * sizeof(PairDesc), cudaMemcpyHostToDevice, g_ctx->stream));
        CK(cudaStreamSynchronize(g_ctx->stream));
    }
    return GX_OK;
}
GX_GUARD_END

int gx_band_upload(gx_band *b, const uint8_t *s1, const uint8_t *s2) try {
    std::lock_guard<std::recursive_mutex> lk(g_mu);
    if (!b) return GX_ERR_ARG;
    if (b->trivial) return GX_OK;
    if (!s1 || !s2) return GX_ERR_ARG;
    const int nl = b->last - b->first;
    const uint64_t c_lo = b->col0[0], c_hi = b->col0[nl - 1] + b->width[nl - 1];
    std::vector<uint8_t> blob(b->m + (c_hi - c_lo));
    memcpy(blob.data(), s1, b->m);
    memcpy(blob.data() + b->m, s2 + c_lo, c_hi - c_lo);
    std::vector<uint64_t> off1(nl, 0), off2(nl);
    for (int q = 0; q < nl; ++q) off2[q] = b->m + (b->col0[q] - c_lo);
    return gx_plan_upload(b->plan, blob.data(), blob.size(), off1.data(), off2.data());
}
GX_GUARD_END

int gx_band_execute(gx_band *b) try {
    std::lock_guard<std::recursive_mutex> lk(g_mu);
    if (!b) return GX_ERR_ARG;
    if (b->trivial) return GX_OK;
    if (!b->connected) return GX_ERR_ARG;
    int rc = gx_plan_execute(b->plan);
    b->fill_ms = b->plan->fill_ms;
    return rc;
}
GX_GUARD_END

int gx_band_score(gx_band *b, int64_t *score, int *valid) try {
    std::lock_guard<std::recursive_mutex> lk(g_mu);
    if (!b || !score || !valid) return GX_ERR_ARG;
    *valid = (b->last == b->n_bands) ? 1 : 0;
    *score = 0;
    if (!*valid) return GX_OK;
    if (b->trivial) {
        const uint64_t len = b->m + b->n_total;
        *score = len ? (int64_t)b->sc.h + (int64_t)len * b->sc.g : 0;
        return GX_OK;
    }
    if (!b->plan->executed) return GX_ERR_ARG;
    const int nl = b->last - b->first;
    std::vector<int64_t> sc(nl);
    int rc = gx_plan_fetch_scores(b->plan, sc.data());
    if (rc) return rc;
    *score = sc[nl - 1];
    return GX_OK;
}
GX_GUARD_END

double gx_band_stat(const gx_band *b, int what) {
    if (!b) return -1.0;
    if (what == 16) return (double)b->epoch;
    if (!b->plan) return what == 3 ? (double)((b->m + 1) * (b->n_total + 1)) : 0.0;
    return gx_plan_stat(b->plan, what);
}

void gx_band_destroy(gx_band *b) {
    std::lock_guard<std::recursive_mutex> lk(g_mu);
    band_free(b);
}

static gx_band *g_band_cache = nullptr;
static void band_cache_drop() {
    if (g_band_cache) band_free(g_band_cache);
    g_band_cache = nullptr;
}

int gx_nw_score_banded(const uint8_t *s1, uint64_t m, const uint8_t *s2, uint64_t n, gx_scores sc, int n_bands, int64_t *score) try {
    std::lock_guard<std::recursive_mutex> lk(g_mu);
    if (!score || (!s1 && m) || (!s2 && n)) return GX_ERR_ARG;
    gx_band *b = g_band_cache;
    const bool hit = b && b->m == m && b->n_total == n && b->n_bands == n_bands && b->first == 0 && b->last == n_bands &&
                     memcmp(&b->sc, &sc, sizeof sc) == 0 && !b->poisoned;
    if (!hit) {
        band_cache_drop();
        b = nullptr;
        int rc = gx_band_create(m, n, n_bands, 0, n_bands, sc, &b);
        if (rc) return rc;
        g_band_cache = b;
    }
    int valid = 0;
    int rc = gx_band_upload(b, s1, s2);
    if (!rc) rc = gx_band_execute(b);
    if (!rc) rc = gx_band_score(b, score, &valid);
    if (rc) band_cache_drop();
    return rc;
}
GX_GUARD_END

int gx_debug_planes(const uint8_t *s1, uint64_t m, const uint8_t *s2, uint64_t n, gx_scores sc, int is_local, int64_t *ins,
                    int64_t *del, int64_t *sub) try {
    std::lock_guard<std::recursive_mutex> lk(g_mu);
    if (!ins || !del || !sub || (!s1 && m) || (!s2 && n)) return GX_ERR_ARG;
    if (!g_ctx) return GX_ERR_NOT_INIT;
    if (!(m < 200 && n < 2000)) return GX_ERR_RANGE;
    int rc = check_scores_impl(sc, m, n, is_local != 0);
    if (rc) return rc;
    Ctx *c = g_ctx;
    CK(cudaSetDevice(c->device));
    const size_t cells = (size_t)(m + 1) * (n + 1);
    uint8_t *d_seq = nullptr;
    long long *d_planes = nullptr;
    rc = pool_alloc(c, m + n + 16, (void **)&d_seq);
    if (!rc) rc = pool_alloc(c, 3 * cells * 8, (void **)&d_planes);
    if (!rc) {
        cudaError_t e = cudaSuccess;
        if (m) e = cudaMemcpyAsync(d_seq, s1, m, cudaMemcpyHostToDevice, c->stream);
        if (e == cudaSuccess && n) e = cudaMemcpyAsync(d_seq + m, s2, n, cudaMemcpyHostToDevice, c->stream);
        if (e == cudaSuccess) {
            PlanesParams pp;
            pp.s1 = d_seq;
            pp.s2 = d_seq + m;
            pp.m = (uint32_t)m;
            pp.n = (uint32_t)n;
            pp.a = sc.s_match;
            pp.b = sc.s_mismatch;
            pp.g = sc.g;
            pp.h = sc.h;
            pp.is_local = is_local ? 1 : 0;
            pp.pi = d_planes;
            pp.pd = d_planes + cells;
            pp.ps = d_planes + 2 * cells;
            gx_planes_kernel<<<1, 256, 0, c->stream>>>(pp);
            e = cudaGetLastError();
        }
        if (e == cudaSuccess) e = cudaMemcpyAsync(ins, d_planes, cells * 8, cudaMemcpyDeviceToHost, c->stream);
        if (e == cudaSuccess) e = cudaMemcpyAsync(del, d_planes + cells, cells * 8, cudaMemcpyDeviceToHost, c->stream);
        if (e == cudaSuccess) e = cudaMemcpyAsync(sub, d_planes + 2 * cells, cells * 8, cudaMemcpyDeviceToHost, c->stream);
        if (e == cudaSuccess) e = cudaStreamSynchronize(c->stream);
        if (e != cudaSuccess) rc = fail_cuda(e, "gx_debug_planes");
    }
    pool_free(c, d_seq);
    pool_free(c, d_planes);
    return rc;
}
GX_GUARD_END

static gx_plan *g_plan_cache = nullptr;
static void plan_cache_drop() {
    if (g_plan_cache) gx_plan_destroy(g_plan_cache);
    g_plan_cache = nullptr;
}
static int cached_plan(const uint64_t *len1, const uint64_t *len2, uint64_t n_pairs, gx_scores sc, int is_local, int flags, gx_plan **out) {
    gx_plan *pl = g_plan_cache;
    const Tunables now = read_tunables();
    if (pl && pl->n_pairs == n_pairs && pl->is_local == (is_local ? 1 : 0) && pl->flags == flags && memcmp(&pl->sc, &sc, sizeof sc) == 0 &&
        memcmp(&pl->tun, &now, sizeof now) == 0 && (n_pairs == 0 || (len1 && len2 && memcmp(pl->len1.data(), len1, n_pairs * 8) == 0 &&
                                                                     memcmp(pl->len2.data(), len2, n_pairs * 8) == 0))) {
        *out = pl;
        return GX_OK;
    }
    plan_cache_drop();
    int rc = gx_plan_create(len1, len2, n_pairs, sc, is_local, flags, &pl);
    if (rc) return rc;
    g_plan_cache = pl;
    *out = pl;
    return GX_OK;
}

int gx_align_batch(const uint8_t *seq_blob, uint64_t blob_len, const uint64_t *off1, const uint64_t *len1, const uint64_t *off2,
                   const uint64_t *len2, uint64_t n_pairs, gx_scores sc, int is_local, int flags, gx_result *out,
                   uint8_t *ops_blob, const uint64_t *ops_off) try {
    std::lock_guard<std::recursive_mutex> lk(g_mu);
    gx_plan *pl = nullptr;
    int rc = cached_plan(len1, len2, n_pairs, sc, is_local, flags, &pl);
    if (rc) return rc;
    rc = gx_plan_upload(pl, seq_blob, blob_len, off1, off2);
    if (!rc) rc = gx_plan_execute(pl);
    if (!rc) rc = gx_plan_fetch(pl, out, ops_blob, ops_off);
    if (rc) plan_cache_drop();
    return rc;
}
GX_GUARD_END

int gx_score_batch(const uint8_t *seq_blob, uint64_t blob_len, const uint64_t *off1, const uint64_t *len1, const uint64_t *off2,
                   const uint64_t *len2, uint64_t n_pairs, gx_scores sc, int is_local, int64_t *scores) try {
    if ((!seq_blob && blob_len) || ((!off1 || !len1 || !off2 || !len2 || !scores) && n_pairs)) return GX_ERR_ARG;
    if (!getenv("GX_NO_STREAM")) {
        const int rcs = score_batch_streamed(seq_blob, blob_len, off1, len1, off2, len2, n_pairs, sc, is_local, scores,
                                             getenv("GX_READS32") != nullptr);
        if (rcs != GX_ERR_UNSUPPORTED) return rcs;
    }
    std::lock_guard<std::recursive_mutex> lk(g_mu);
    gx_plan *pl = nullptr;
    int rc = cached_plan(len1, len2, n_pairs, sc, is_local, 0, &pl);
    if (rc) return rc;
    rc = gx_plan_upload(pl, seq_blob, blob_len, off1, off2);
    if (!rc) rc = gx_plan_execute(pl);
    if (!rc) rc = gx_plan_fetch_scores(pl, scores);
    if (rc) plan_cache_drop();
    return rc;
}
GX_GUARD_END

int gx_align_pair(const uint8_t *s1, uint64_t m, const uint8_t *s2, uint64_t n, gx_scores sc, int is_local, int flags,
                  gx_result *out, uint8_t *ops, uint64_t ops_cap) try {
    if (!out || (!s1 && m) || (!s2 && n)) return GX_ERR_ARG;
    if (m > (1ull << 28) || n > (1ull << 28)) return GX_ERR_RANGE;
    if ((flags & GX_FLAG_TRACEBACK) && (!ops || ops_cap < m + n + 1)) return (!ops) ? GX_ERR_ARG : GX_ERR_OPS_CAP;
    std::vector<uint8_t> blob(m + n);
    if (m) memcpy(blob.data(), s1, m);
    if (n) memcpy(blob.data() + m, s2, n);
    uint64_t off1 = 0, off2 = m, l1 = m, l2 = n;
    uint64_t ops_off[2] = {0, ops_cap};
    return gx_align_batch(blob.data(), m + n, &off1, &l1, &off2, &l2, 1, sc, is_local, flags, out, ops, ops_off);
}
GX_GUARD_END

}
```

### genomics_rs_b200/csrc/gx_common.cuh

```cuda
#pragma once
#include <cuda_runtime.h>
#include <stdint.h>

namespace gx {

constexpr int NEG32 = -(1 << 30);

#ifndef GX_PANEL_LOG2
#define GX_PANEL_LOG2 12
#endif
constexpr int PANEL_H_LOG2 = GX_PANEL_LOG2;
constexpr int PANEL_H = 1 << PANEL_H_LOG2;
constexpr int WARPS_PER_CTA = 8;
constexpr int CTA_THREADS = WARPS_PER_CTA * 32;
__host__ __device__ constexpr int ctas_per_sm(int K) { return K > 0 ? 2 : 2; }
__host__ __device__ constexpr int warps_per_sm(int K) { return WARPS_PER_CTA * ctas_per_sm(K); }

constexpr int WARP_SMEM_S1 = PANEL_H + 32;
constexpr int WARP_SMEM_BYTES = WARP_SMEM_S1 + 512 + 512 + 16;
__host__ __device__ constexpr int warp_smem_bytes(int ) { return WARP_SMEM_BYTES; }

#ifdef GX_CHECKED
#define GX_CHECK(word, cond, site)                                   \
    do {                                                             \
        if (!(cond)) atomicMax(reinterpret_cast<unsigned int *>(word), (unsigned int)(site)); \
    } while (0)
#else
#define GX_CHECK(word, cond, site) ((void)0)
#endif

struct PairDesc {
    uint64_t s1_off, s2_off;
    uint64_t colbuf_off;
    uint64_t top_off;
    uint64_t codes_off;
    uint64_t ops_off;
    uint32_t m, n;
    uint32_t S, P;
    uint32_t progress_off;
    uint32_t tile_base;
    uint32_t tile_code_bytes;
    uint32_t col0;
    const unsigned long long *inbox;
    unsigned long long *outbox;
    const uint32_t *ack;
};

__host__ inline bool tile_in_code_band(uint64_t m, uint64_t n, uint32_t p, uint32_t s, uint32_t W, uint64_t code_w) {
    const uint64_t i0 = (uint64_t)p << PANEL_H_LOG2;
    const uint64_t i1 = (i0 + PANEL_H < m) ? i0 + PANEL_H : m;
    const uint64_t lo = i0 * n / m, hi = i1 * n / m;
    const uint64_t c0 = (uint64_t)s * W, c1 = c0 + W;
    return c1 + code_w > lo && c0 < hi + code_w + 1;
}

struct TileDesc {
    uint32_t pair, p, s, pad_;
};

struct DevResult {
    long long score;
    unsigned long long start_i, start_j, end_i, end_j, n_ops, matches, mismatches, gap_extensions, opening_gaps, lcs_at_first_max;
    double fill_ms, walk_ms;
};

struct FillParams {
    const uint8_t *blob;
    const uint8_t *blob_sym;
    uint32_t one;
    const PairDesc *pairs;
    const TileDesc *tiles;
    uint32_t n_pairs;
    uint32_t n_tiles;
    uint32_t pmax;
    uint32_t parity;
    uint32_t cpb;
    uint32_t epoch;
    uint32_t *ticket;
    uint32_t *progress;
    unsigned long long *colbuf;
    int2 *top;
    uint8_t *codes;
    const uint8_t *tile_codes;
    uint64_t code_bytes;
    int4 *tile_best;
    uint32_t pad_keys;
    uint32_t poll_nap;
    uint32_t start_lead;
    unsigned long long *timeline;
    unsigned long long *stats;
    int g, hg, ap, bp, h;
};

struct WalkParams {
    const uint8_t *blob;
    const PairDesc *pairs;
    uint32_t n_pairs;
    const int2 *top;
    const uint8_t *codes;
    const int4 *tile_best;
    DevResult *results;
    uint8_t *ops;
    int g, hg, h;
    int kcols_log2;
    int is_local, traceback, have_best;
    int debug;
    uint32_t *left_band;
    const uint8_t *tile_codes;
    uint32_t *check;
    uint64_t code_bytes, ops_bytes;
    uint32_t win_rows;
};

__device__ __forceinline__ uint32_t smem_u32(const void *p) { return (uint32_t)__cvta_generic_to_shared(p); }

__device__ __forceinline__ void mbar_init(uint64_t *bar, uint32_t count) {
    asm volatile("mbarrier.init.shared::cta.b64 [%0], %1;" ::"r"(smem_u32(bar)), "r"(count) : "memory");
}
__device__ __forceinline__ void mbar_expect_tx(uint64_t *bar, uint32_t bytes) {
    asm volatile("mbarrier.arrive.expect_tx.shared::cta.b64 _, [%0], %1;" ::"r"(smem_u32(bar)), "r"(bytes) : "memory");
}
__device__ __forceinline__ bool mbar_try_wait(uint64_t *bar, uint32_t phase) {
    uint32_t ok;
    asm volatile(
        "{\n\t.reg .pred p;\n\t"
        "mbarrier.try_wait.parity.shared::cta.b64 p, [%1], %2;\n\t"
        "selp.u32 %0, 1, 0, p;\n\t}"
        : "=r"(ok)
        : "r"(smem_u32(bar)), "r"(phase)
        : "memory");
    return ok != 0;
}
__device__ __forceinline__ void tma_bulk_g2s(void *dst_smem, const void *src_gmem, uint32_t bytes, uint64_t *bar) {
    asm volatile("cp.async.bulk.shared::cluster.global.mbarrier::complete_tx::bytes [%0], [%1], %2, [%3];" ::"r"(smem_u32(dst_smem)),
                 "l"(src_gmem), "r"(bytes), "r"(smem_u32(bar))
                 : "memory");
}
__device__ __forceinline__ void fence_proxy_async_smem() { asm volatile("fence.proxy.async.shared::cta;" ::: "memory"); }
__device__ __forceinline__ void fence_mbar_init() { asm volatile("fence.mbarrier_init.release.cluster;" ::: "memory"); }

__device__ __forceinline__ unsigned long long ld_relaxed_u64(const unsigned long long *p) {
    unsigned long long v;
    asm volatile("ld.relaxed.gpu.global.u64 %0, [%1];" : "=l"(v) : "l"(p) : "memory");
    return v;
}
__device__ __forceinline__ void st_relaxed_u64(unsigned long long *p, unsigned long long v) {
    asm volatile("st.relaxed.gpu.global.u64 [%0], %1;" ::"l"(p), "l"(v) : "memory");
}
__device__ __forceinline__ unsigned long long ld_relaxed_sys_u64(const unsigned long long *p) {
    unsigned long long v;
    asm volatile("ld.relaxed.sys.global.u64 %0, [%1];" : "=l"(v) : "l"(p) : "memory");
    return v;
}
__device__ __forceinline__ void st_relaxed_sys_u64(unsigned long long *p, unsigned long long v) {
    asm volatile("st.relaxed.sys.global.u64 [%0], %1;" ::"l"(p), "l"(v) : "memory");
}
__device__ __forceinline__ uint32_t ld_acquire_sys_u32(const uint32_t *p) {
    uint32_t v;
    asm volatile("ld.acquire.sys.global.u32 %0, [%1];" : "=r"(v) : "l"(p) : "memory");
    return v;
}
__device__ __forceinline__ void st_release_sys_u32(uint32_t *p, uint32_t v) {
    asm volatile("st.release.sys.global.u32 [%0], %1;" ::"l"(p), "r"(v) : "memory");
}
__device__ __forceinline__ uint32_t ld_relaxed_u32(const uint32_t *p) {
    uint32_t v;
    asm volatile("ld.relaxed.gpu.global.u32 %0, [%1];" : "=r"(v) : "l"(p) : "memory");
    return v;
}
__device__ __forceinline__ uint32_t ld_acquire_u32(const uint32_t *p) {
    uint32_t v;
    asm volatile("ld.acquire.gpu.global.u32 %0, [%1];" : "=r"(v) : "l"(p) : "memory");
    return v;
}
__device__ __forceinline__ void st_release_u32(uint32_t *p, uint32_t v) {
    asm volatile("st.release.gpu.global.u32 [%0], %1;" ::"l"(p), "r"(v) : "memory");
}
__device__ __forceinline__ int2 ld_cg_int2(const int2 *p) {
    int2 v;
    asm volatile("ld.global.cg.v2.s32 {%0,%1}, [%2];" : "=r"(v.x), "=r"(v.y) : "l"(p) : "memory");
    return v;
}
__device__ __forceinline__ void st_cg_int2(int2 *p, int2 v) {
    asm volatile("st.global.cg.v2.s32 [%0], {%1,%2};" ::"l"(p), "r"(v.x), "r"(v.y) : "memory");
}
__device__ __forceinline__ void st_cs_uint4(uint4 *p, uint4 v) {
    asm volatile("st.global.cs.v4.u32 [%0], {%1,%2,%3,%4};" ::"l"(p), "r"(v.x), "r"(v.y), "r"(v.z), "r"(v.w) : "memory");
}

__device__ __forceinline__ uint2 lds_volatile_uint2(const uint2 *p) {
    uint2 v;
    asm volatile("ld.volatile.shared.v2.u32 {%0,%1}, [%2];" : "=r"(v.x), "=r"(v.y) : "r"(smem_u32(p)) : "memory");
    return v;
}

__device__ __forceinline__ unsigned long long globaltimer_ns() {
    unsigned long long t;
    asm volatile("mov.u64 %0, %%globaltimer;" : "=l"(t));
    return t;
}

template <int N>
struct Log2 {
    static constexpr int value = 1 + Log2<N / 2>::value;
};
template <>
struct Log2<1> {
    static constexpr int value = 0;
};

}
```

### genomics_rs_b200/csrc/gx_fill.cuh

```cuda
#pragma once
#include <type_traits>

#include "gx_common.cuh"

namespace gx {

constexpr unsigned FULL = 0xffffffffu;
constexpr uint32_t SPIN_LIMIT = 1u << 22;

__device__ __forceinline__ bool spin_check(uint32_t &spins, uint32_t *abort_word) {
    if (++spins > SPIN_LIMIT) atomicExch(abort_word, 1u);
    if ((spins & 63u) == 0u || spins > SPIN_LIMIT) {
        if (*reinterpret_cast<volatile uint32_t *>(abort_word) != 0u) return true;
    }
    return false;
}

template <int N, class F>
__device__ __forceinline__ void static_for(F &&f) {
    if constexpr (N > 0) {
        static_for<N - 1>(f);
        f(std::integral_constant<int, N - 1>{});
    }
}

template <uint32_t UNIT>
__device__ __forceinline__ void code_acc(uint32_t &cw, int S, int I, int V, uint32_t one) {
    asm("{\n\t.reg .pred p1, p2;\n\t"
        "setp.ne.s32 p1, %1, %3;\n\t"
        "setp.ne.and.s32 p2, %2, %3, p1;\n\t"
        "@p1 mad.lo.u32 %0, %4, %5, %0;\n\t"
        "@p2 mad.lo.u32 %0, %4, %5, %0;\n\t}"
        : "+r"(cw)
        : "r"(S), "r"(I), "r"(V), "r"(one), "n"(UNIT));
}

#ifndef GX_SCORE_CTAS
#define GX_SCORE_CTAS 2
#endif
template <int K, int R>
struct Geo {
    static_assert(R * K <= 64 && (R & (R - 1)) == 0 && (K & (K - 1)) == 0, "R x K cells must fit one 16-byte code chunk");
    static constexpr int W = 32 * K;
    static constexpr int SPC = 64 / (R * K);
    static constexpr int CPB_MAX = 32 / (SPC * R) > 0 ? 32 / (SPC * R) : 1;
    static constexpr int KB = Log2<K>::value;
    static_assert(SPC * R <= 32, "one chunk must not exceed 32 rows");
};
__host__ __device__ __forceinline__ uint32_t tile_batches(uint32_t rows, uint32_t R, uint32_t batch) {
    return ((rows + R - 1) / R + 31 + batch - 1) / batch;
}

__device__ __forceinline__ void lds_over_if(int &x, int &y, const uint2 *p, bool pred) {
    asm volatile("{\n\t.reg .pred q;\n\tsetp.ne.u32 q, %3, 0;\n\t@q ld.shared.v2.u32 {%0,%1}, [%2];\n\t}"
                 : "+r"(x), "+r"(y)
                 : "r"(smem_u32(p)), "r"((uint32_t)pred));
}

template <int K, int R, bool LOCAL, bool CODES, int TRACK, bool PROF, bool MASKED, bool PAD, bool CHAIN1, bool THRU = false>
__device__ __forceinline__ void run_batch(int (&eu)[K], int (&du)[K], const int (&c2)[K], int (&eo)[R], int (&io)[R], int &vd,
                                          int &best, int &best_r, const int g, const int hg, const int ap, const int bp,
                                          const uint32_t one, const uint8_t *s1base ,
                                          const int (&prof4)[K] ,
                                          const uint2 *inr , uint2 *outring, uint4 *code_dst,
                                          const int t0, const int rows, const int lane, const int kvalid,
                                          int (&c1a)[R] , const int cpb ,
                                          uint32_t *chk , const int s1lo, const int s1hi ) {
    using G = Geo<K, R>;
    constexpr int KB = G::KB;
    const bool lane0 = lane == 0;
    auto s1char = [&](int r) __attribute__((always_inline)) -> int {
        if (MASKED) return (int)s1base[min(max(r, 0), rows - 1)];
        GX_CHECK(chk, r >= s1lo && r < s1hi, 11);
        return (int)s1base[r];
    };
#pragma unroll 1
    for (int ch = 0; ch < cpb; ++ch) {
        uint32_t cw[4] = {0u, 0u, 0u, 0u};
        int rbk[(TRACK == 2 || TRACK == 3) ? G::SPC * R : 1];
        static_for<G::SPC>([&](auto uc) {
            constexpr int uu = decltype(uc)::value;
            const int step = ch * G::SPC + uu;
            const int rb = t0 + step - lane;
            const int r0 = rb * R;
            int el[R], il[R];
#pragma unroll
            for (int rr = 0; rr < R; ++rr) {
                el[rr] = __shfl_up_sync(FULL, eo[rr], 1);
                il[rr] = __shfl_up_sync(FULL, io[rr], 1);
                GX_CHECK(chk, step * R + rr >= 0 && step * R + rr < 32, 12);
#ifdef GX_LDS_SEL
                {
                    const uint2 bnd = inr[step * R + rr];
                    el[rr] = lane0 ? (int)bnd.x : el[rr];
                    il[rr] = lane0 ? (int)bnd.y : il[rr];
                }
#else
                lds_over_if(el[rr], il[rr], inr + step * R + rr, lane0);
#endif
            }
            bool act[R];
#pragma unroll
            for (int rr = 0; rr < R; ++rr) act[rr] = MASKED ? ((r0 + rr >= 0) && (r0 + rr < rows)) : true;
            int c1[R];
#pragma unroll
            for (int rr = 0; rr < R; ++rr) {
                c1[rr] = PROF ? (int)(1u << c1a[rr]) : c1a[rr];
                c1a[rr] = s1char(r0 + R + rr);
            }
            int e_[R], i_[R], ed_[R], mh_[R], rowbest[R];
#pragma unroll
            for (int rr = 0; rr < R; ++rr) {
                e_[rr] = el[rr];
                i_[rr] = il[rr];
                ed_[rr] = (rr == 0) ? vd : el[rr > 0 ? rr - 1 : 0];
                mh_[rr] = el[rr];
                rowbest[rr] = (CHAIN1 || TRACK == 3) ? INT32_MIN : -1;
            }
            static_for<R + K - 1>([&](auto dc) {
                constexpr int d = decltype(dc)::value;
                static_for<R>([&](auto rc) {
                    constexpr int rr = decltype(rc)::value;
                    constexpr int k = d - rr;
                    if constexpr (k >= 0 && k < K) {
                        int In, Dn, En, Skey, Ikey, Vkey;
                        if (CHAIN1) {
                            In = LOCAL ? __viaddmax_s32_relu(i_[rr], g, mh_[rr]) : __viaddmax_s32(i_[rr], g, mh_[rr]);
                            Dn = LOCAL ? __viaddmax_s32_relu(du[k], g, eu[k]) : __viaddmax_s32(du[k], g, eu[k]);
                            const int Sh = PROF ? __dp4a(c1[rr], prof4[k], ed_[rr]) : ed_[rr] + ((c1[rr] == c2[k]) ? ap : bp);
                            const int Mh = __viaddmax_s32(Dn, hg, Sh);
                            En = __viaddmax_s32(In, hg, Mh);
                            if (THRU) mh_[rr] = (k < kvalid) ? Mh : mh_[rr];
                            else mh_[rr] = Mh;
                            Skey = Sh;
                            Ikey = CODES ? In + hg : 0;
                            Vkey = En;
                        } else {
                            In = LOCAL ? __viaddmax_s32_relu(i_[rr], g, e_[rr]) : __viaddmax_s32(i_[rr], g, e_[rr]);
                            Dn = LOCAL ? __viaddmax_s32_relu(du[k], g, eu[k]) : __viaddmax_s32(du[k], g, eu[k]);
                            const int Sn = PROF ? __dp4a(c1[rr], prof4[k], ed_[rr]) : ed_[rr] + ((c1[rr] == c2[k]) ? ap : bp);
                            const int Vn = LOCAL ? __vimax3_s32_relu(In, Dn, Sn) : __vimax3_s32(In, Dn, Sn);
                            En = Vn + hg;
                            Skey = Sn;
                            Ikey = In;
                            Vkey = Vn;
                        }
                        if (CODES) {
                            constexpr int bitpos = ((uu * R + rr) * K + k) * 2;
                            code_acc<(1u << (bitpos & 31))>(cw[bitpos >> 5], Skey, Ikey, Vkey, one);
                        }
                        ed_[rr] = eu[k];
                        if (MASKED) {
                            eu[k] = act[rr] ? En : eu[k];
                            du[k] = act[rr] ? Dn : du[k];
                        } else {
                            eu[k] = En;
                            du[k] = Dn;
                        }
                        if (THRU) {
                            e_[rr] = (k < kvalid) ? En : e_[rr];
                            i_[rr] = (k < kvalid) ? In : i_[rr];
                        } else {
                            e_[rr] = En;
                            i_[rr] = In;
                        }
                        if (TRACK == 2) {
                            int key = (Vkey << KB) | k;
                            if (PAD) key = (k < kvalid) ? key : (CHAIN1 ? INT32_MIN : -1);
                            rowbest[rr] = max(rowbest[rr], key);
                        } else if (TRACK == 1) {
                            int key = Vkey;
                            if (PAD) key = (k < kvalid) ? key : (CHAIN1 ? INT32_MIN : -1);
                            rowbest[rr] = max(rowbest[rr], key);
                        } else if (TRACK == 3) {
                            int key = (Vkey << KB) | (K - 1 - k);
                            if (PAD) key = (k < kvalid) ? key : INT32_MIN;
                            rowbest[rr] = max(rowbest[rr], key);
                        }
                    }
                });
            });
            if (MASKED) vd = act[0] ? el[R - 1] : vd;
            else vd = el[R - 1];
#pragma unroll
            for (int rr = 0; rr < R; ++rr) {
                eo[rr] = e_[rr];
                io[rr] = i_[rr];
                if (TRACK == 2 || TRACK == 3) {
                    rbk[uu * R + rr] = act[rr] ? rowbest[rr] : INT32_MIN;
                } else if (TRACK == 1) {
                    best = act[rr] ? max(best, rowbest[rr]) : best;
                }
                GX_CHECK(chk, step * R + rr < 32, 13);
                if (lane == 31 && act[rr]) outring[step * R + rr] = make_uint2((uint32_t)e_[rr], (uint32_t)i_[rr]);
            }
        });
        if (TRACK == 2 || TRACK == 3) {
            const int rbase = (t0 + ch * G::SPC - lane) * R;
#pragma unroll
            for (int x = 0; x < G::SPC * R; ++x) {
                const bool upd = (TRACK == 2) ? ((rbk[x] | (K - 1)) >= best && rbk[x] != INT32_MIN) : ((rbk[x] | (K - 1)) > (best | (K - 1)));
                best = upd ? rbk[x] : best;
                best_r = upd ? rbase + x : best_r;
            }
        }
        if (CODES) st_cs_uint4(code_dst + ch * 32, make_uint4(cw[0], cw[1], cw[2], cw[3]));
    }
}

template <int K, int R, bool LOCAL, bool CODES, int TRACK, bool PROF, bool CHAIN1, bool BAND = false>
__global__ void __launch_bounds__(CTA_THREADS, CODES ? ctas_per_sm(K) : GX_SCORE_CTAS) gx_fill_kernel(const FillParams P) {
    using G = Geo<K, R>;
    constexpr int W = G::W;
    const int cpb = (int)P.cpb;
    const int B = cpb * G::SPC;
    const int BR = B * R;
    constexpr int KB = G::KB;
    extern __shared__ __align__(16) uint8_t smem[];
    const int lane = threadIdx.x & 31;
    const int wib = threadIdx.x >> 5;
    uint8_t *wsm = smem + wib * warp_smem_bytes(K);
    uint8_t *s1buf = wsm;
    uint2 *inring = reinterpret_cast<uint2 *>(wsm + WARP_SMEM_S1);
    uint2 *outring = inring + 64;
    uint64_t *mbar = reinterpret_cast<uint64_t *>(outring + 64);
    static_assert(WARP_SMEM_S1 + 2 * 64 * 8 + 16 == WARP_SMEM_BYTES, "per-warp shared-memory layout");

    for (int x = lane; x < WARP_SMEM_S1 / 16; x += 32) reinterpret_cast<uint4 *>(s1buf)[x] = make_uint4(0u, 0u, 0u, 0u);
    if (lane == 0) {
        mbar_init(mbar, 1);
        fence_mbar_init();
    }
    __syncwarp();
    uint32_t phase = 0;
    const int g = P.g, hg = P.hg, h = P.h;
    const int ap = CHAIN1 ? P.ap + P.hg : P.ap, bp = CHAIN1 ? P.bp + P.hg : P.bp;
    const uint32_t one = P.one;
    const uint32_t parity = P.parity;
    uint32_t *abort_word = P.ticket + 1;
    uint32_t *chk = P.ticket + 2;
    (void)chk;
    bool dead = false;
    const uint8_t *seq = PROF ? P.blob_sym : P.blob;

    const uint32_t wg = blockIdx.x * (blockDim.x >> 5) + (uint32_t)wib;
    uint32_t own = 0;
    for (;;) {
        uint32_t tk = 0;
        if (P.pmax != 0u) {
            if (own >= P.pmax) break;
            tk = wg * P.pmax + own++;
        } else {
            if (lane == 0) tk = atomicAdd(P.ticket, 1u);
            tk = __shfl_sync(FULL, tk, 0);
        }
        if (tk >= P.n_tiles) break;
        const TileDesc td = P.tiles[tk];
        if (td.pair == 0xffffffffu) break;
        GX_CHECK(chk, td.pair < P.n_pairs, 1);
        const long long st_t0 = P.stats ? clock64() : 0;
        const unsigned long long tl_take = P.stats ? globaltimer_ns() : 0ull;
        unsigned long long tl_dp0 = 0ull;
        long long st_top = 0, st_bnd = 0, st_s1 = 0;
        const PairDesc *pd = P.pairs + td.pair;
        const int m = (int)pd->m, n = (int)pd->n, S = (int)pd->S;
        const int p = (int)td.p, s = (int)td.s;
        const int i0 = p << PANEL_H_LOG2;
        const int rows = min(PANEL_H, m - i0);
        const int jl = s * W + lane * K;
        const int kvalid = min(max(n - jl, 0), K);
        const bool has_pad = (s + 1) * W > n;
        const int col0 = (int)pd->col0;
        GX_CHECK(chk, p >= 0 && p < (int)pd->P && s >= 0 && s < S && rows > 0 && rows <= PANEL_H, 2);
        GX_CHECK(chk, BR >= 1 && BR <= 32 && cpb >= 1 && cpb <= G::CPB_MAX, 3);

        const uint8_t *s1g = seq + pd->s1_off + i0;
        const uint32_t delta = (uint32_t)(reinterpret_cast<uintptr_t>(s1g) & 15u);
        __syncwarp();
        if (lane == 0) {
            fence_proxy_async_smem();
            const uint32_t bytes = (delta + (uint32_t)rows + 15u) & ~15u;
            mbar_expect_tx(mbar, bytes);
            tma_bulk_g2s(s1buf, s1g - delta, bytes, mbar);
        }

        int c2[K];
        {
            const uint8_t *s2g = seq + pd->s2_off + jl;
#pragma unroll
            for (int k = 0; k < K; ++k) c2[k] = (k < kvalid) ? (int)__ldg(s2g + k) : 256;
        }
        int prof4[K];
#pragma unroll
        for (int k = 0; k < K; ++k) {
            uint32_t w = 0u;
#pragma unroll
            for (int sym = 0; sym < 4; ++sym) w |= ((uint32_t)((c2[k] == 8 * sym) ? ap : bp) & 0xffu) << (8 * sym);
            prof4[k] = PROF ? (int)w : 0;
        }

        int eu[K], du[K];
        if (p == 0) {
#pragma unroll
            for (int k = 0; k < K; ++k) {
                eu[k] = (LOCAL ? 0 : h + (col0 + jl + k + 1) * g) + hg;
                du[k] = NEG32;
            }
        } else {
            const uint32_t *pr = P.progress + pd->progress_off + s;
            uint32_t spins = 0;
            const long long w0 = P.stats ? clock64() : 0;
            uint32_t nap = 100;
            while (ld_relaxed_u32(pr) < (uint32_t)p) {
                if (spin_check(spins, abort_word)) {
                    dead = true;
                    break;
                }
                __nanosleep(nap);
                nap = min(nap * 2u, 1000u);
            }
            (void)ld_acquire_u32(pr);
            if (P.stats) st_top += clock64() - w0;
            if (dead) break;
            const int2 *tp = P.top + pd->top_off + jl;
#pragma unroll
            for (int k = 0; k < K; ++k) {
                int2 v = make_int2(NEG32, NEG32);
                if (k < kvalid) v = ld_cg_int2(tp + k);
                eu[k] = v.x;
                du[k] = v.y;
            }
        }
        const bool left_band = (s == 0) && (pd->inbox != nullptr);
        const bool right_band = (s == S - 1) && (pd->outbox != nullptr);
        const unsigned long long *cb_in =
            (s > 0) ? P.colbuf + pd->colbuf_off + (uint64_t)(s - 1) * m + i0 : (left_band ? pd->inbox + i0 : nullptr);
        unsigned long long *cb_out =
            (s < S - 1) ? P.colbuf + pd->colbuf_off + (uint64_t)s * m + i0 : (right_band ? pd->outbox + i0 : nullptr);
        const bool has_left = cb_in != nullptr;
        auto ld_bnd = [&](const unsigned long long *q) __attribute__((always_inline)) { return left_band ? ld_relaxed_sys_u64(q) : ld_relaxed_u64(q); };

        int vd = __shfl_up_sync(FULL, eu[K - 1], 1);
        if (lane == 0) {
            if (!has_left) {
                vd = ((p == 0) ? 0 : (LOCAL ? 0 : h + i0 * g)) + hg;
            } else if (p == 0) {
                vd = (LOCAL ? 0 : h + (col0 + jl) * g) + hg;
            } else {
                unsigned long long v;
                uint32_t spins = 0;
                while ((((uint32_t)((v = ld_bnd(cb_in - 1)) >> 32)) & 1u) != parity) {
                    if (spin_check(spins, abort_word)) {
                        dead = true;
                        break;
                    }
                    __nanosleep(100);
                }
                vd = (int)(uint32_t)v;
            }
        }
        if (right_band && p == 0 && pd->ack != nullptr && lane == 0) {
            uint32_t spins = 0;
            while (ld_acquire_sys_u32(pd->ack) + 1u < P.epoch) {
                if (spin_check(spins, abort_word)) {
                    dead = true;
                    break;
                }
                __nanosleep(2000);
            }
        }
        dead = __any_sync(FULL, dead);
        if (dead) break;

        int eo[R], io[R];
#pragma unroll
        for (int rr = 0; rr < R; ++rr) eo[rr] = io[rr] = 0;
        int best = (CHAIN1 || TRACK == 3) ? INT32_MIN : -1, best_r = 0;
        const uint32_t nbat = tile_batches((uint32_t)rows, R, B);
        uint4 *code_base = nullptr;
        if (CODES)
            code_base = reinterpret_cast<uint4 *>(P.codes + pd->codes_off + (uint64_t)(p * S + s) * pd->tile_code_bytes) + lane;
        bool tcodes = CODES;
        if constexpr (BAND) tcodes = P.tile_codes[pd->tile_base + p * S + s] != 0;

        unsigned long long nxt = 0;
        auto issue = [&](uint32_t bt) __attribute__((always_inline)) {
            const int r = (int)(BR * bt) + lane;
            GX_CHECK(chk, !(has_left && lane < BR && r < rows) || (i0 + r >= 0 && i0 + r < m), 4);
            if (has_left && lane < BR && r < rows) nxt = ld_bnd(cb_in + r);
        };
        if (has_left && P.start_lead > 0) {
            const int lead = min((int)P.start_lead, rows - 1);
            uint32_t spins = 0;
            const long long w0 = P.stats ? clock64() : 0;
            while ((((uint32_t)(ld_bnd(cb_in + lead) >> 32)) & 1u) != parity) {
                if (spin_check(spins, abort_word)) {
                    dead = true;
                    break;
                }
                __nanosleep(500);
            }
            if (P.stats) st_bnd += clock64() - w0;
            dead = __any_sync(FULL, dead);
            if (dead) break;
        }
        issue(0);

        {
            uint32_t tries = 0;
            const long long w0 = P.stats ? clock64() : 0;
            while (!mbar_try_wait(mbar, phase)) {
                if (++tries > (1u << 24)) {
                    atomicExch(abort_word, 1u);
                    dead = true;
                    break;
                }
            }
            dead = __any_sync(FULL, dead);
            if (P.stats) st_s1 += clock64() - w0;
            if (dead) break;
        }
        phase ^= 1u;
        const uint8_t *s1base = s1buf + delta;
        __syncwarp();
        int c1a[R];
#pragma unroll
        for (int rr = 0; rr < R; ++rr) c1a[rr] = s1base[min(max(-lane * R + rr, 0), rows - 1)];

        const bool lane_b = lane < BR;
        auto settle = [&](uint32_t b) __attribute__((always_inline)) -> bool {
            const int rb = (int)(BR * b) + lane;
            const bool need = has_left && lane_b && (rb < rows);
            bool ok = !need || ((((uint32_t)(nxt >> 32)) & 1u) == parity);
            if (!__all_sync(FULL, ok)) {
                uint32_t spins = 0;
                const long long w0 = P.stats ? clock64() : 0;
                bool lost = false;
                do {
                    if (__any_sync(FULL, spin_check(spins, abort_word))) {
                        lost = true;
                        break;
                    }
                    if (P.poll_nap) __nanosleep(P.poll_nap);
                    if (!ok) nxt = ld_bnd(cb_in + rb);
                    ok = !need || ((((uint32_t)(nxt >> 32)) & 1u) == parity);
                } while (!__all_sync(FULL, ok));
                if (P.stats) st_bnd += clock64() - w0;
                if (lost) return false;
            }
            uint2 cur;
            cur.x = has_left ? (uint32_t)nxt : (uint32_t)((LOCAL ? 0 : h + (i0 + rb + 1) * g) + hg);
            cur.y = has_left ? (uint32_t)(((int)(uint32_t)(nxt >> 32)) >> 1) : (uint32_t)NEG32;
            GX_CHECK(chk, !lane_b || (b & 1u) * BR + lane < 64, 5);
            if (lane_b) inring[(b & 1u) * BR + lane] = cur;
            return true;
        };
        if (!settle(0)) dead = true;
        if (nbat > 1) issue(1);
        __syncwarp();
        if (P.stats) tl_dp0 = globaltimer_ns();
        uint2 pub = make_uint2(0u, 0u);
        int pub_row = -1;
        auto flush_pub = [&]() __attribute__((always_inline)) {
            if (pub_row >= 0) {
                GX_CHECK(chk, i0 + pub_row < m, 6);
                const unsigned long long packed =
                    (unsigned long long)pub.x | ((unsigned long long)((pub.y << 1) | parity) << 32);
                if (right_band) st_relaxed_sys_u64(cb_out + pub_row, packed);
                else st_relaxed_u64(cb_out + pub_row, packed);
            }
        };
        const bool has_out = cb_out != nullptr;
        auto post = [&](uint32_t bt, uint2 *outr) __attribute__((always_inline)) -> bool {
            const int ro = ((int)(B * bt) - 31) * R + lane;
            const bool take = has_out && lane_b && ro >= 0 && ro < rows;
            __syncwarp();
            if (take) pub = lds_volatile_uint2(outr + lane);
            pub_row = take ? ro : -1;
            flush_pub();
            pub_row = -1;
            if (bt + 1 < nbat) {
                if (!settle(bt + 1)) return false;
                if (bt + 2 < nbat) issue(bt + 2);
                __syncwarp();
            }
            return true;
        };
        const uint32_t nb_head = (30 + B) / B;
        const uint32_t nb_body = max(nb_head, ((uint32_t)rows / R) / B);
        bool thru = false;
        if constexpr (!LOCAL && !CODES && TRACK == 0) thru = right_band && has_pad;
        auto run_tile = [&](auto codes_c) __attribute__((always_inline)) {
            constexpr bool WC = decltype(codes_c)::value;
            uint32_t bt = 0;
            for (int ph = 0; ph < 2 && !dead; ++ph) {
                const uint32_t m_end = (ph == 0 && !thru) ? min(nb_head, nbat) : nbat;
                for (; bt < m_end && !dead; ++bt) {
                    uint2 *outr = outring + (bt & 1u) * BR;
                    uint4 *cdst = WC ? code_base + (size_t)bt * cpb * 32 : nullptr;
                    GX_CHECK(chk, !WC || ((size_t)(bt + 1) * cpb * 512 <= pd->tile_code_bytes &&
                                          pd->codes_off + (uint64_t)(p * S + s + 1) * pd->tile_code_bytes <= P.code_bytes), 7);
                    if constexpr (!LOCAL && !CODES && TRACK == 0) {
                        if (thru)
                            run_batch<K, R, LOCAL, WC, TRACK, PROF, true, false, CHAIN1, true>(eu, du, c2, eo, io, vd, best, best_r, g, hg, ap, bp,
                                                                                            one, s1base, prof4, inring + (bt & 1u) * BR, outr, cdst,
                                                                                            (int)(B * bt), rows, lane, kvalid, c1a, cpb, chk, -(int)delta, WARP_SMEM_S1 - (int)delta);
                    }
                    if (!thru)
                        run_batch<K, R, LOCAL, WC, TRACK, PROF, true, (TRACK != 0), CHAIN1>(eu, du, c2, eo, io, vd, best, best_r, g, hg, ap, bp,
                                                                                         one, s1base, prof4, inring + (bt & 1u) * BR, outr, cdst,
                                                                                         (int)(B * bt), rows, lane, kvalid, c1a, cpb, chk, -(int)delta, WARP_SMEM_S1 - (int)delta);
                    if (!post(bt, outr)) dead = true;
                }
                if (ph != 0 || thru || dead) continue;
                if ((TRACK != 0) && has_pad && P.pad_keys != 0u) {
                    for (; bt < nb_body && !dead; ++bt) {
                        uint2 *outr = outring + (bt & 1u) * BR;
                        uint4 *cdst = WC ? code_base + (size_t)bt * cpb * 32 : nullptr;
                        GX_CHECK(chk, !WC || ((size_t)(bt + 1) * cpb * 512 <= pd->tile_code_bytes &&
                                              pd->codes_off + (uint64_t)(p * S + s + 1) * pd->tile_code_bytes <= P.code_bytes), 7);
                        run_batch<K, R, LOCAL, WC, TRACK, PROF, false, true, CHAIN1>(eu, du, c2, eo, io, vd, best, best_r, g, hg, ap, bp,
                                                                                  one, s1base, prof4, inring + (bt & 1u) * BR, outr, cdst,
                                                                                  (int)(B * bt), rows, lane, kvalid, c1a, cpb, chk, -(int)delta, WARP_SMEM_S1 - (int)delta);
                        if (!post(bt, outr)) dead = true;
                    }
                } else {
                    for (; bt < nb_body && !dead; ++bt) {
                        uint2 *outr = outring + (bt & 1u) * BR;
                        uint4 *cdst = WC ? code_base + (size_t)bt * cpb * 32 : nullptr;
                        GX_CHECK(chk, !WC || ((size_t)(bt + 1) * cpb * 512 <= pd->tile_code_bytes &&
                                              pd->codes_off + (uint64_t)(p * S + s + 1) * pd->tile_code_bytes <= P.code_bytes), 7);
                        run_batch<K, R, LOCAL, WC, TRACK, PROF, false, false, CHAIN1>(eu, du, c2, eo, io, vd, best, best_r, g, hg, ap, bp,
                                                                                   one, s1base, prof4, inring + (bt & 1u) * BR, outr, cdst,
                                                                                   (int)(B * bt), rows, lane, kvalid, c1a, cpb, chk, -(int)delta, WARP_SMEM_S1 - (int)delta);
                        if (!post(bt, outr)) dead = true;
                    }
                }
            }
        };
        if constexpr (BAND) {
            if (tcodes) run_tile(std::true_type{});
            else run_tile(std::false_type{});
        } else {
            run_tile(std::integral_constant<bool, CODES>{});
        }
        flush_pub();
        if (dead) break;

        {
            int2 *tp = P.top + pd->top_off + jl;
#pragma unroll
            for (int k = 0; k < K; ++k) {
                GX_CHECK(chk, !(k < kvalid) || jl + k < n, 8);
                if (k < kvalid) st_cg_int2(tp + k, make_int2(eu[k], du[k]));
            }
            __syncwarp();
            if (lane == 0) st_release_u32(P.progress + pd->progress_off + s, (uint32_t)(p + 1));
        }

        if (TRACK != 0) {
            int bv, bi, bj;
            if (TRACK == 2) {
                if (CHAIN1) bv = (kvalid == 0) ? -1 : (best >> KB) - hg;
                else bv = (best < 0) ? -1 : (best >> KB);
                bi = i0 + best_r + 1;
                bj = jl + (best & (K - 1)) + 1;
            } else if (TRACK == 3) {
                bv = (kvalid == 0) ? INT32_MIN : (best >> KB) - (CHAIN1 ? hg : 0);
                bi = i0 + best_r + 1;
                bj = jl + (K - 1 - (best & (K - 1))) + 1;
            } else {
                if (CHAIN1) bv = (kvalid == 0) ? -1 : best - hg;
                else bv = best;
                bi = 0;
                bj = 0;
            }
#pragma unroll
            for (int off = 16; off > 0; off >>= 1) {
                const int ov = __shfl_xor_sync(FULL, bv, off);
                const int oi = __shfl_xor_sync(FULL, bi, off);
                const int oj = __shfl_xor_sync(FULL, bj, off);
                const bool take = (TRACK == 3) ? ((ov > bv) || (ov == bv && (oi < bi || (oi == bi && oj < bj))))
                                               : ((ov > bv) || (ov == bv && (oi > bi || (oi == bi && oj > bj))));
                bv = take ? ov : bv;
                bi = take ? oi : bi;
                bj = take ? oj : bj;
            }
            if (lane == 0) P.tile_best[pd->tile_base + p * S + s] = make_int4(bv, bi, bj, 0);
        }
        if (P.stats && lane == 0) {
            atomicAdd(P.stats + 0, (unsigned long long)st_top);
            atomicAdd(P.stats + 1, (unsigned long long)st_bnd);
            atomicAdd(P.stats + 2, (unsigned long long)(clock64() - st_t0));
            atomicAdd(P.stats + 3, (unsigned long long)st_s1);
            atomicAdd(P.stats + 4, 1ull);
            if (P.timeline) {
                unsigned long long *tl = P.timeline + 4ull * tk;
                uint32_t smid;
                asm volatile("mov.u32 %0, %%smid;" : "=r"(smid));
                tl[0] = tl_take;
                tl[1] = tl_dp0;
                tl[2] = globaltimer_ns();
                tl[3] = ((unsigned long long)td.pair << 48) | ((unsigned long long)p << 32) | ((unsigned long long)s << 12) | smid;
            }
        }
    }
}

static __global__ void __launch_bounds__(256) gx_encode_kernel(const uint8_t *__restrict__ in, uint8_t *__restrict__ out, size_t n,
                                                        const uint8_t *__restrict__ lut256) {
    __shared__ uint8_t lut[256];
    lut[threadIdx.x] = lut256[threadIdx.x];
    __syncthreads();
    for (size_t i = (size_t)blockIdx.x * blockDim.x + threadIdx.x; i < n; i += (size_t)gridDim.x * blockDim.x) out[i] = lut[in[i]];
}

static __global__ void gx_band_ack_kernel(uint32_t *peer_ack, uint32_t epoch) { st_release_sys_u32(peer_ack, epoch); }

}
```

### include/gxalign.h

```cpp
#ifndef GXALIGN_H
#define GXALIGN_H

#include <stdint.h>

#ifdef __cplusplus
extern "C" {
#endif

enum {
    GX_OK = 0,
    GX_ERR_ARG = 1,
    GX_ERR_SCORES = 2,
    GX_ERR_RANGE = 3,
    GX_ERR_OPS_CAP = 4,
    GX_ERR_NO_DEVICE = 5,
    GX_ERR_CUDA = 6,
    GX_ERR_NOMEM = 7,
    GX_ERR_NOT_INIT = 8,
    GX_ERR_UNSUPPORTED = 9,
    GX_ERR_INTERNAL = 10
};

typedef struct gx_scores {
    int32_t s_match;
    int32_t s_mismatch;
    int32_t g;
    int32_t h;
} gx_scores;

enum {
    GX_MATCH = 0, GX_MISMATCH = 1, GX_INSERT = 2, GX_DELETE = 3, GX_OPEN_INSERT = 4, GX_OPEN_DELETE = 5
};

enum {
    GX_FLAG_TRACEBACK = 1,
    GX_FLAG_LCS_AT_MAX = 2,
    GX_FLAG_START_CELL = 4
};

typedef struct gx_result {
    int64_t score;
    uint64_t start_i, start_j;
    uint64_t end_i, end_j;
    uint64_t n_ops;
    uint64_t matches, mismatches, gap_extensions, opening_gaps;
    uint64_t lcs_at_first_max;
    double fill_ms, walk_ms;
} gx_result;

int gx_init(int device);
void gx_shutdown(void);
int gx_device_count(void);
const char *gx_strerror(int status);
const char *gx_last_error(void);
const char *gx_version(void);

int gx_check_scores(gx_scores sc, uint64_t m, uint64_t n);

int gx_align_pair(const uint8_t *s1, uint64_t m, const uint8_t *s2, uint64_t n,
                  gx_scores sc, int is_local, int flags,
                  gx_result *out, uint8_t *ops, uint64_t ops_cap);

int gx_align_batch(const uint8_t *seq_blob, uint64_t blob_len,
                   const uint64_t *off1, const uint64_t *len1,
                   const uint64_t *off2, const uint64_t *len2, uint64_t n_pairs,
                   gx_scores sc, int is_local, int flags,
                   gx_result *out, uint8_t *ops_blob, const uint64_t *ops_off);

int gx_score_batch(const uint8_t *seq_blob, uint64_t blob_len,
                   const uint64_t *off1, const uint64_t *len1,
                   const uint64_t *off2, const uint64_t *len2, uint64_t n_pairs,
                   gx_scores sc, int is_local, int64_t *scores);

typedef struct gx_plan gx_plan;
int gx_plan_create(const uint64_t *len1, const uint64_t *len2, uint64_t n_pairs,
                   gx_scores sc, int is_local, int flags, gx_plan **plan);
int gx_plan_upload(gx_plan *plan, const uint8_t *seq_blob, uint64_t blob_len,
                   const uint64_t *off1, const uint64_t *off2);
int gx_plan_execute(gx_plan *plan);
int gx_plan_fetch(gx_plan *plan, gx_result *out, uint8_t *ops_blob, const uint64_t *ops_off);
int gx_plan_fetch_scores(gx_plan *plan, int64_t *scores);
void gx_plan_destroy(gx_plan *plan);
double gx_plan_stat(const gx_plan *plan, int what);
int gx_plan_debug_timeline(gx_plan *plan, uint64_t *out, uint64_t cap_words);

#define GX_BAND_HANDLE_BYTES 64
typedef struct gx_band gx_band;
int gx_band_range(uint64_t n_total, int n_bands, int band, uint64_t *col0, uint64_t *width);
int gx_band_create(uint64_t m, uint64_t n_total, int n_bands, int first_band, int last_band, gx_scores sc, gx_band **band);
int gx_band_export(gx_band *band, void *handle, uint64_t handle_cap);
int gx_band_connect(gx_band *band, const void *left_handle, const void *right_handle);
int gx_band_upload(gx_band *band, const uint8_t *s1, const uint8_t *s2);
int gx_band_execute(gx_band *band);
int gx_band_score(gx_band *band, int64_t *score, int *valid);
double gx_band_stat(const gx_band *band, int what);
void gx_band_destroy(gx_band *band);
int gx_nw_score_banded(const uint8_t *s1, uint64_t m, const uint8_t *s2, uint64_t n, gx_scores sc, int n_bands, int64_t *score);

int gx_debug_planes(const uint8_t *s1, uint64_t m, const uint8_t *s2, uint64_t n, gx_scores sc, int is_local,
                    int64_t *insert_scores, int64_t *delete_scores, int64_t *sub_scores);

int gx_debug_tile_order(const uint64_t *len1, const uint64_t *len2, uint64_t n_pairs, int K, int bands, uint32_t *out,
                        uint64_t cap_tiles, uint64_t *n_tiles);

int gx_replay_ops(const uint8_t *ops, uint64_t n_ops, uint64_t start_i, uint64_t start_j,
                  uint32_t *ops_i, uint32_t *ops_j);

int gx_k0_measure(double *out, int n);

#ifdef __cplusplus
}
#endif
#endif
```

Measured before the change: 2945.

## Fill paired out-of-band tiles of two alignments at once with packed 16-bit SIMD

Adds a dual-tile fill path. Pairs of alignments sorted by length are matched up, and for interior tiles outside the traceback code band both partners' tiles are processed together in one warp. Their DP values are packed as offset 16-bit halves and updated with paired s16x2 instructions (viaddmax, prmt). A frame check on the score parameters guards against overflow, and the base is rebased every batch. The aim is to double cell throughput on score-only tiles, at the cost of extra shared memory per warp, extra host-side ticket building and more branching in the kernel.

```diff
diff --git a/genomics_rs_b200/_lib.py b/genomics_rs_b200/_lib.py
--- a/genomics_rs_b200/_lib.py
+++ b/genomics_rs_b200/_lib.py
@@ -18,6 +18,7 @@
     "gx_plan_fetch", "gx_plan_fetch_scores", "gx_plan_destroy", "gx_plan_stat", "gx_plan_debug_timeline", "gx_replay_ops", "gx_k0_measure",
     "gx_band_range", "gx_band_create", "gx_band_export", "gx_band_connect", "gx_band_upload", "gx_band_execute",
     "gx_band_score", "gx_band_stat", "gx_band_destroy", "gx_nw_score_banded", "gx_debug_planes", "gx_debug_tile_order",
+    "gx_debug_dual_order", "gx_dual_frame_ok",
 ]
 
 
@@ -94,6 +95,8 @@
         lib.gx_nw_score_banded.argtypes = [vp, u64, vp, u64, GxScores, i32, C.POINTER(C.c_int64)]
         lib.gx_nw_score_banded.restype = i32
         lib.gx_debug_tile_order.argtypes = [vp, vp, u64, i32, i32, vp, u64, C.POINTER(u64)]; lib.gx_debug_tile_order.restype = i32
+        lib.gx_debug_dual_order.argtypes = [vp, vp, u64, i32, vp, u64, C.POINTER(u64)]; lib.gx_debug_dual_order.restype = i32
+        lib.gx_dual_frame_ok.argtypes = [GxScores, i32, i32]; lib.gx_dual_frame_ok.restype = i32
         lib.gx_debug_planes.argtypes = [vp, u64, vp, u64, GxScores, i32, vp, vp, vp]; lib.gx_debug_planes.restype = i32
         _lib = lib
     return _lib
diff --git a/genomics_rs_b200/csrc/gx_api.cu b/genomics_rs_b200/csrc/gx_api.cu
--- a/genomics_rs_b200/csrc/gx_api.cu
+++ b/genomics_rs_b200/csrc/gx_api.cu
@@ -120,6 +120,7 @@
 
 struct Tunables {
     int r = -1, batch = -1, code_band = -1, band_resident = 1;
+    int dual = 1;
     int k = -1, chain1 = -1, tickets = -1, resident = -1, wpc = -1, grid_cap = -1, pad_keys = 0, poll_nap = 0, start_lead = 0,
         fill_stats = 0, walk_stats = 0, walk_rows = 0, no_stream = 0, reads32 = 0, test_abort = 0;
 };
@@ -134,6 +135,7 @@
     t.batch = env_int("GX_BATCH", -1);
     t.band_resident = env_int("GX_BAND_RESIDENT", 1);
     t.code_band = env_int("GX_CODE_BAND", -1);
+    t.dual = env_int("GX_DUAL", 1);
     t.chain1 = env_int("GX_CHAIN1", -1);
     t.tickets = getenv("GX_TICKETS") ? 1 : -1;
     t.resident = env_int("GX_RESIDENT", -1);
@@ -172,6 +174,7 @@
     std::vector<gx::PairDesc> pairs;
     std::vector<uint64_t> len1, len2;
     uint64_t n_tiles = 0;
+    uint64_t n_list = 0;
     uint64_t n_strips = 0;
     uint64_t cells = 0;
     uint64_t code_bytes = 0, ops_bytes = 0, colbuf_entries = 0, top_entries = 0, progress_entries = 0, best_entries = 0;
@@ -215,6 +218,11 @@
     int band_fallbacks = 0;
     uint32_t left_band = 0;
     double code_cell_frac = 1.0;
+    bool dual_ok = false;
+    bool tiles_dual = false;
+    std::vector<uint8_t> h_tile_codes;
+    std::vector<int64_t> partner;
+    double dual_cell_frac = 0.0;
     uint64_t h2d_bytes = 0, d2h_bytes = 0, dev_bytes = 0;
     gx_band *band = nullptr;
 };
@@ -272,8 +280,9 @@
     int wpc = (pl->n_strips * 2 >= (uint64_t)c->sm_count * warps_per_sm(K)) ? WARPS_PER_CTA : 1;
     if (pl->tun.wpc >= 0) wpc = pl->tun.wpc == 1 ? 1 : WARPS_PER_CTA;
     if (pl->resident) wpc = 1;
-    const size_t smem = (size_t)wpc * warp_smem_bytes(K);
-    CK(cudaFuncSetAttribute(kern, cudaFuncAttributeMaxDynamicSharedMemorySize, (int)(WARPS_PER_CTA * warp_smem_bytes(K))));
+    const uint32_t wsm = (uint32_t)warp_smem_bytes(K) + ((banded && pl->tiles_dual) ? (uint32_t)WARP_SMEM_S1 : 0u);
+    const size_t smem = (size_t)wpc * wsm;
+    CK(cudaFuncSetAttribute(kern, cudaFuncAttributeMaxDynamicSharedMemorySize, (int)(WARPS_PER_CTA * wsm)));
     int occ = 0;
     CK(cudaOccupancyMaxActiveBlocksPerMultiprocessor(&occ, kern, wpc * 32, smem));
     if (occ < 1) occ = 1;
@@ -282,6 +291,7 @@
     uint64_t cap = (uint64_t)c->sm_count * occ;
     FillParams fq = fp;
     fq.tile_codes = banded ? pl->d_tile_codes : nullptr;
+    fq.wsm = wsm;
     if (pl->resident && pl->n_strips > cap) {
         g_err = "resident-strips plan does not fit the device (fewer than 16 single-warp CTAs per SM)";
         return GX_ERR_INTERNAL;
@@ -291,7 +301,7 @@
         fq.tiles = pl->d_strips;
         fq.n_tiles = (uint32_t)(pl->n_strips * pl->pmax);
     }
-    uint64_t want = fq.pmax ? pl->n_strips : (pl->n_tiles + wpc - 1) / wpc;
+    uint64_t want = fq.pmax ? pl->n_strips : (pl->n_list + wpc - 1) / wpc;
     if (pl->tun.grid_cap >= 0) grid_cap = pl->tun.grid_cap;
     if (grid_cap > 0 && (uint64_t)grid_cap < cap) cap = grid_cap;
     int grid = (int)std::min<uint64_t>(want, cap);
@@ -499,8 +509,10 @@
 }
 
 
+static uint32_t no_dual(uint32_t, uint32_t, uint32_t) { return 0u; }
+template <class Dual = decltype(&no_dual)>
 static void build_ticket_order(const std::vector<uint32_t> &S, const std::vector<uint32_t> &P, const std::vector<uint64_t> &sbase,
-                               std::vector<TileDesc> &tiles) {
+                               std::vector<TileDesc> &tiles, Dual dual = &no_dual) {
     const size_t n_pairs = S.size();
     constexpr uint64_t TS = PANEL_H / 64;
     uint64_t vmax = 0;
@@ -520,10 +532,66 @@
             const uint64_t sv = v - sbase[q];
             const uint64_t p_hi = std::min<uint64_t>(P[q] - 1, sv / TS);
             const uint64_t p_lo = (sv >= S[q]) ? (sv - S[q] + 1 + TS - 1) / TS : 0;
-            for (uint64_t p2 = p_lo; p2 <= p_hi; ++p2) tiles.push_back({q, (uint32_t)p2, (uint32_t)(sv - TS * p2), 0});
+            for (uint64_t p2 = p_lo; p2 <= p_hi; ++p2) {
+                const uint32_t s2 = (uint32_t)(sv - TS * p2), d = dual(q, (uint32_t)p2, s2);
+                if (d == 0u || d - 1u > q) tiles.push_back({q, (uint32_t)p2, s2, d});
+            }
         }
         live.resize(keep);
     }
+}
+
+static double code_band_flags(const std::vector<PairDesc> &pairs, uint32_t W, int code_w, std::vector<uint8_t> &flags) {
+    double with = 0, all = 0;
+    for (const PairDesc &pd : pairs) {
+        const uint64_t dmn = pd.m > pd.n ? pd.m - pd.n : pd.n - pd.m;
+        const uint64_t cw = code_w > 0 ? (uint64_t)code_w : 1024 + dmn;
+        for (uint32_t p2 = 0; p2 < pd.P; ++p2) {
+            const double rows = (double)std::min<uint64_t>(PANEL_H, pd.m - (uint64_t)p2 * PANEL_H);
+            for (uint32_t s2 = 0; s2 < pd.S; ++s2) {
+                const double cols = (double)std::min<uint64_t>((uint64_t)W, pd.n - (uint64_t)s2 * W);
+                const bool in = tile_in_code_band(pd.m, pd.n, p2, s2, W, cw);
+                flags[pd.tile_base + (uint64_t)p2 * pd.S + s2] = in ? 1 : 0;
+                all += rows * cols;
+                if (in) with += rows * cols;
+            }
+        }
+    }
+    return all > 0 ? with / all : 1.0;
+}
+
+static std::vector<int64_t> dual_partners(const std::vector<PairDesc> &pairs) {
+    std::vector<uint32_t> idx;
+    for (uint32_t q = 0; q < (uint32_t)pairs.size(); ++q)
+        if (pairs[q].S && pairs[q].P) idx.push_back(q);
+    std::stable_sort(idx.begin(), idx.end(), [&](uint32_t x, uint32_t y) {
+        return pairs[x].m != pairs[y].m ? pairs[x].m < pairs[y].m : pairs[x].n < pairs[y].n;
+    });
+    std::vector<int64_t> partner(pairs.size(), -1);
+    for (size_t k = 0; k + 1 < idx.size(); k += 2) {
+        partner[idx[k]] = idx[k + 1];
+        partner[idx[k + 1]] = idx[k];
+    }
+    return partner;
+}
+static uint32_t dual_of(const std::vector<PairDesc> &pairs, const std::vector<uint8_t> &flags, const std::vector<int64_t> &partner,
+                        uint32_t q, uint32_t p, uint32_t s) {
+    if (partner[q] < 0) return 0u;
+    const PairDesc &a = pairs[q], &b = pairs[(size_t)partner[q]];
+    auto single_ok = [&](const PairDesc &d) {
+        return ((uint64_t)p + 1) * PANEL_H <= d.m && s + 1 < d.S && flags[d.tile_base + (uint64_t)p * d.S + s] == 0;
+    };
+    return (single_ok(a) && single_ok(b)) ? (uint32_t)partner[q] + 1u : 0u;
+}
+
+static bool dual_frame_ok(gx_scores sc, int K, uint32_t batch_steps) {
+    const long long a = sc.s_match, b = sc.s_mismatch, g = sc.g, hg = (long long)sc.h + sc.g;
+    if (a - hg < 0 || a - hg > 127 || b - hg < 0 || b - hg > 127) return false;
+    if (batch_steps != 32u || K < 1) return false;
+    const long long delta = std::max(std::max(a, b) - hg, -hg);
+    const long long span = 32ll * K + 2 * 32 + 4;
+    const long long M = delta * span + 2 * (-hg) + std::max(std::llabs(a), std::llabs(b)) + (-g);
+    return M < DUAL_OFF - 64;
 }
 
 static int plan_create_locked(const uint64_t *len1, const uint64_t *len2, uint64_t n_pairs, gx_scores sc, int is_local, int flags,
@@ -697,6 +765,7 @@
         build_ticket_order(Sv, Pv, sbase, tiles);
     }
     pl->n_tiles = n_tiles_total;
+    pl->n_list = tiles.size();
     std::vector<TileDesc> strips;
     {
         if (pl->resident) {
@@ -732,26 +801,15 @@
     std::vector<uint8_t> tile_codes;
     if (pl->traceback && !is_local && !band_col0 && (!pl->resident || pl->tun.band_resident != 0) && pl->tun.code_band != 0 && best > 0) {
         tile_codes.assign(best, 1);
-        double with = 0, all = 0;
-        for (uint64_t q = 0; q < n_pairs; ++q) {
-            const PairDesc &pd = pl->pairs[q];
-            const uint64_t dmn = pd.m > pd.n ? pd.m - pd.n : pd.n - pd.m;
-            const uint64_t cw = pl->tun.code_band > 0 ? (uint64_t)pl->tun.code_band : 1024 + dmn;
-            for (uint32_t p2 = 0; p2 < pd.P; ++p2) {
-                const double rows = (double)std::min<uint64_t>(PANEL_H, pd.m - (uint64_t)p2 * PANEL_H);
-                for (uint32_t s2 = 0; s2 < pd.S; ++s2) {
-                    const double cols = (double)std::min<uint64_t>((uint64_t)W, pd.n - (uint64_t)s2 * W);
-                    const bool in = tile_in_code_band(pd.m, pd.n, p2, s2, (uint32_t)W, cw);
-                    tile_codes[pd.tile_base + (uint64_t)p2 * pd.S + s2] = in ? 1 : 0;
-                    all += rows * cols;
-                    if (in) with += rows * cols;
-                }
-            }
-        }
-        pl->code_cell_frac = all > 0 ? with / all : 1.0;
+        pl->code_cell_frac = code_band_flags(pl->pairs, (uint32_t)W, pl->tun.code_band, tile_codes);
         pl->code_band = pl->code_cell_frac < 0.9;
         if (!pl->code_band) pl->code_cell_frac = 1.0;
         if (pl->code_band) A(best, (void **)&pl->d_tile_codes);
+    }
+    pl->dual_ok = pl->code_band && !pl->lcs && !pl->resident && !pl->chain1 && K == 8 && R == 1 && pl->tun.dual != 0 && dual_frame_ok(sc, K, BATCH);
+    if (pl->dual_ok) {
+        pl->h_tile_codes = tile_codes;
+        pl->partner = dual_partners(pl->pairs);
     }
     if (pl->traceback) A(ops, (void **)&pl->d_ops);
     if (rc == GX_OK && pl->code_band) {
@@ -961,6 +1019,8 @@
     return plan_create_locked(len1, len2, n_pairs, sc, is_local, flags, nullptr, out);
 }
 GX_GUARD_END
+
+static int plan_set_dual(gx_plan *pl);
 
 int gx_plan_upload(gx_plan *pl, const uint8_t *blob, uint64_t blob_len, const uint64_t *off1, const uint64_t *off2) try {
     std::lock_guard<std::recursive_mutex> lk(g_mu);
@@ -1049,6 +1109,10 @@
         }
     }
     CK(cudaStreamSynchronize(c->stream));
+    if (pl->kind == KIND_WAVEFRONT) {
+        int rc = plan_set_dual(pl);
+        if (rc) return rc;
+    }
     pl->uploaded = true;
     return GX_OK;
 }
@@ -1056,7 +1120,7 @@
 
 static int plan_execute_once(gx_plan *pl, bool *aborted);
 
-static int plan_build_tickets(gx_plan *pl) {
+static int plan_build_tickets(gx_plan *pl, bool dual = false) {
     Ctx *c = pl->ctx;
     const size_t np = pl->pairs.size();
     std::vector<uint32_t> Sv(np), Pv(np);
@@ -1070,8 +1134,26 @@
     }
     std::vector<TileDesc> tiles;
     tiles.reserve(pl->n_tiles);
-    build_ticket_order(Sv, Pv, sbase, tiles);
-    if (tiles.size() != pl->n_tiles) return GX_ERR_INTERNAL;
+    uint64_t covered = 0;
+    double dual_cells = 0;
+    if (dual) {
+        build_ticket_order(Sv, Pv, sbase, tiles,
+                           [&](uint32_t q, uint32_t p, uint32_t s) { return dual_of(pl->pairs, pl->h_tile_codes, pl->partner, q, p, s); });
+        for (const TileDesc &t : tiles) {
+            covered += t.pad_ ? 2 : 1;
+            if (t.pad_) dual_cells += 2.0 * PANEL_H * 32.0 * pl->K;
+        }
+        double all = 0;
+        for (const PairDesc &pd : pl->pairs) all += (double)pd.m * pd.n;
+        dual_cells = all > 0 ? dual_cells / all : 0.0;
+    } else {
+        build_ticket_order(Sv, Pv, sbase, tiles);
+        covered = tiles.size();
+    }
+    if (covered != pl->n_tiles) return GX_ERR_INTERNAL;
+    pl->tiles_dual = dual;
+    pl->dual_cell_frac = dual_cells;
+    pl->n_list = tiles.size();
     if (tiles.empty()) return GX_OK;
     pool_free(c, pl->d_tiles);
     pl->d_tiles = nullptr;
@@ -1080,6 +1162,11 @@
     CK(cudaMemcpyAsync(pl->d_tiles, tiles.data(), tiles.size() * sizeof(TileDesc), cudaMemcpyHostToDevice, c->stream));
     CK(cudaStreamSynchronize(c->stream));
     return GX_OK;
+}
+
+static int plan_set_dual(gx_plan *pl) {
+    const bool want = pl->dual_ok && pl->code_band && pl->prof && !pl->resident;
+    return want == pl->tiles_dual ? GX_OK : plan_build_tickets(pl, want);
 }
 
 int gx_plan_execute(gx_plan *pl) try {
@@ -1102,6 +1189,8 @@
         pl->code_band = false;
         pl->code_cell_frac = 1.0;
         pl->band_fallbacks++;
+        int rb = plan_set_dual(pl);
+        if (rb) return rb;
         rc = plan_execute_once(pl, &aborted);
         pl->fill_ms += f0;
         pl->walk_ms += w0;
@@ -1196,7 +1285,7 @@
     fp.n_pairs = (uint32_t)pl->n_pairs;
     fp.code_bytes = pl->code_bytes;
     fp.tiles = pl->d_tiles;
-    fp.n_tiles = (uint32_t)pl->n_tiles;
+    fp.n_tiles = (uint32_t)pl->n_list;
     fp.pmax = 0;
     fp.parity = pl->parity;
     fp.cpb = pl->cpb;
@@ -1431,6 +1520,46 @@
 }
 GX_GUARD_END
 
+int gx_debug_dual_order(const uint64_t *len1, const uint64_t *len2, uint64_t n_pairs, int code_w, uint32_t *out,
+                        uint64_t cap_entries, uint64_t *n_entries) try {
+    if ((!len1 || !len2) && n_pairs) return GX_ERR_ARG;
+    if (!n_entries) return GX_ERR_ARG;
+    constexpr uint32_t W = 32 * 8;
+    std::vector<PairDesc> pairs(n_pairs);
+    std::vector<uint32_t> S(n_pairs), P(n_pairs);
+    std::vector<uint64_t> sbase(n_pairs, 0);
+    uint64_t best = 0;
+    for (uint64_t q = 0; q < n_pairs; ++q) {
+        PairDesc &pd = pairs[q];
+        memset(&pd, 0, sizeof pd);
+        const bool interior = len1[q] > 0 && len2[q] > 0;
+        pd.m = (uint32_t)len1[q];
+        pd.n = (uint32_t)len2[q];
+        pd.S = S[q] = interior ? (uint32_t)((len2[q] + W - 1) / W) : 0;
+        pd.P = P[q] = interior ? (uint32_t)((len1[q] + PANEL_H - 1) / PANEL_H) : 0;
+        pd.tile_base = (uint32_t)best;
+        best += (uint64_t)pd.S * pd.P;
+    }
+    std::vector<uint8_t> flags(best, 1);
+    code_band_flags(pairs, W, code_w, flags);
+    const std::vector<int64_t> partner = dual_partners(pairs);
+    std::vector<TileDesc> tiles;
+    build_ticket_order(S, P, sbase, tiles, [&](uint32_t q, uint32_t p, uint32_t s) { return dual_of(pairs, flags, partner, q, p, s); });
+    *n_entries = tiles.size();
+    if (!out) return GX_OK;
+    if (cap_entries < tiles.size()) return GX_ERR_ARG;
+    for (size_t k = 0; k < tiles.size(); ++k) {
+        out[4 * k + 0] = tiles[k].pair;
+        out[4 * k + 1] = tiles[k].p;
+        out[4 * k + 2] = tiles[k].s;
+        out[4 * k + 3] = tiles[k].pad_;
+    }
+    return GX_OK;
+}
+GX_GUARD_END
+
+int gx_dual_frame_ok(gx_scores sc, int K, int batch_steps) { return (batch_steps > 0 && dual_frame_ok(sc, K, (uint32_t)batch_steps)) ? 1 : 0; }
+
 double gx_plan_stat(const gx_plan *pl, int what) {
     if (!pl) return -1.0;
     switch (what) {
@@ -1455,6 +1584,7 @@
         case 18: return pl->lcs_ms;
         case 25: return pl->prof ? 1.0 : 0.0;
         case 26: return (double)pl->reads_bits;
+        case 27: return pl->tiles_dual ? pl->dual_cell_frac : 0.0;
         case 10: case 11: case 12: case 13: case 14: return (double)pl->h_stats[what - 10];
         default: return -1.0;
     }
diff --git a/genomics_rs_b200/csrc/gx_common.cuh b/genomics_rs_b200/csrc/gx_common.cuh
--- a/genomics_rs_b200/csrc/gx_common.cuh
+++ b/genomics_rs_b200/csrc/gx_common.cuh
@@ -75,6 +75,7 @@
     uint32_t pmax;
     uint32_t parity;
     uint32_t cpb;
+    uint32_t wsm;
     uint32_t epoch;
     uint32_t *ticket;
     uint32_t *progress;
diff --git a/genomics_rs_b200/csrc/gx_fill.cuh b/genomics_rs_b200/csrc/gx_fill.cuh
--- a/genomics_rs_b200/csrc/gx_fill.cuh
+++ b/genomics_rs_b200/csrc/gx_fill.cuh
@@ -208,6 +208,72 @@
     }
 }
 
+constexpr int DUAL_OFF = 1 << 14;
+
+__device__ __forceinline__ uint32_t dual_pack(int a, int b) {
+    return (uint32_t)max(a, 0) | ((uint32_t)max(b, 0) << 16);
+}
+__device__ __forceinline__ int dual_lo(uint32_t x) { return (int)(x & 0xffffu) - DUAL_OFF; }
+__device__ __forceinline__ int dual_hi(uint32_t x) { return (int)(x >> 16) - DUAL_OFF; }
+__device__ __forceinline__ bool dual_in_frame(uint32_t x) { return (x & 0x80008000u) == 0u; }
+__device__ __forceinline__ uint32_t dual_sel(uint32_t a8, uint32_t b8) { return (a8 >> 3) * 0x11u + (b8 >> 3) * 0x1100u + 0xC480u; }
+__device__ __forceinline__ uint32_t prmt(uint32_t x, uint32_t y, uint32_t s) {
+    uint32_t d;
+    asm("prmt.b32 %0, %1, %2, %3;" : "=r"(d) : "r"(x), "r"(y), "r"(s));
+    return d;
+}
+
+template <int K, bool MASKED>
+__device__ __forceinline__ void run_batch_dual(uint32_t (&eu)[K], uint32_t (&du)[K], const uint32_t (&pa)[K], const uint32_t (&pb)[K],
+                                               uint32_t &eo, uint32_t &io, uint32_t &vd, const uint32_t g2, const uint32_t hg2,
+                                               const uint32_t one, const uint8_t *s1a, const uint8_t *s1b, const uint2 *inr,
+                                               uint2 *outring, const int t0, const int rows, const int lane,
+                                               uint32_t &sela , const int cpb, uint32_t *chk) {
+    constexpr int SPC = Geo<K, 1>::SPC;
+    const bool lane0 = lane == 0;
+#pragma unroll 1
+    for (int ch = 0; ch < cpb; ++ch) {
+        static_for<SPC>([&](auto uc) {
+            constexpr int uu = decltype(uc)::value;
+            const int step = ch * SPC + uu;
+            const int r0 = t0 + step - lane;
+            int el = __shfl_up_sync(FULL, (int)eo, 1);
+            int il = __shfl_up_sync(FULL, (int)io, 1);
+            lds_over_if(el, il, inr + step, lane0);
+            const bool act = MASKED ? (r0 >= 0 && r0 < rows) : true;
+            const uint32_t sel = sela;
+            {
+                const int rn = MASKED ? min(max(r0 + 1, 0), rows - 1) : r0 + 1;
+                sela = dual_sel(s1a[rn], s1b[rn]);
+            }
+            uint32_t e_ = (uint32_t)el, i_ = (uint32_t)il, ed = vd;
+#pragma unroll
+            for (int k = 0; k < K; ++k) {
+                const uint32_t In = __viaddmax_s16x2(i_, g2, e_);
+                const uint32_t Dn = __viaddmax_s16x2(du[k], g2, eu[k]);
+                const uint32_t Sn = prmt(pa[k], pb[k], sel) * one + ed;
+                const uint32_t Vn = __vimax3_s16x2(In, Dn, Sn);
+                const uint32_t En = Vn * one + hg2;
+                GX_CHECK(chk, !act || (dual_in_frame(In) && dual_in_frame(Dn) && dual_in_frame(En)), 14);
+                ed = eu[k];
+                if (MASKED) {
+                    eu[k] = act ? En : eu[k];
+                    du[k] = act ? Dn : du[k];
+                } else {
+                    eu[k] = En;
+                    du[k] = Dn;
+                }
+                e_ = En;
+                i_ = In;
+            }
+            vd = act ? (uint32_t)el : vd;
+            eo = e_;
+            io = i_;
+            if (lane == 31 && act) outring[step] = make_uint2(e_, i_);
+        });
+    }
+}
+
 template <int K, int R, bool LOCAL, bool CODES, int TRACK, bool PROF, bool CHAIN1, bool BAND = false>
 __global__ void __launch_bounds__(CTA_THREADS, CODES ? ctas_per_sm(K) : GX_SCORE_CTAS) gx_fill_kernel(const FillParams P) {
     using G = Geo<K, R>;
@@ -216,17 +282,21 @@
     const int B = cpb * G::SPC;
     const int BR = B * R;
     constexpr int KB = G::KB;
+    constexpr bool DUAL = BAND && K == 8 && R == 1 && !CHAIN1 && PROF && !LOCAL;
     extern __shared__ __align__(16) uint8_t smem[];
     const int lane = threadIdx.x & 31;
     const int wib = threadIdx.x >> 5;
-    uint8_t *wsm = smem + wib * warp_smem_bytes(K);
+    uint8_t *wsm = smem + wib * P.wsm;
     uint8_t *s1buf = wsm;
     uint2 *inring = reinterpret_cast<uint2 *>(wsm + WARP_SMEM_S1);
     uint2 *outring = inring + 64;
     uint64_t *mbar = reinterpret_cast<uint64_t *>(outring + 64);
     static_assert(WARP_SMEM_S1 + 2 * 64 * 8 + 16 == WARP_SMEM_BYTES, "per-warp shared-memory layout");
+    uint8_t *s1buf_b = wsm + WARP_SMEM_BYTES;
 
     for (int x = lane; x < WARP_SMEM_S1 / 16; x += 32) reinterpret_cast<uint4 *>(s1buf)[x] = make_uint4(0u, 0u, 0u, 0u);
+    if (DUAL && P.wsm > (uint32_t)WARP_SMEM_BYTES)
+        for (int x = lane; x < WARP_SMEM_S1 / 16; x += 32) reinterpret_cast<uint4 *>(s1buf_b)[x] = make_uint4(0u, 0u, 0u, 0u);
     if (lane == 0) {
         mbar_init(mbar, 1);
         fence_mbar_init();
@@ -245,6 +315,268 @@
 
     const uint32_t wg = blockIdx.x * (blockDim.x >> 5) + (uint32_t)wib;
     uint32_t own = 0;
+
+    auto dual_tile = [&](const TileDesc td, unsigned long long &tl_dp0, long long &st_top, long long &st_bnd,
+                         long long &st_s1) __attribute__((always_inline)) -> bool {
+        GX_CHECK(chk, td.pad_ - 1u < P.n_pairs && td.pad_ - 1u != td.pair, 16);
+        const PairDesc *pa = P.pairs + td.pair, *pb = P.pairs + (td.pad_ - 1u);
+        const int ma = (int)pa->m, mb = (int)pb->m;
+        const int p = (int)td.p, s = (int)td.s;
+        const int i0 = p << PANEL_H_LOG2;
+        constexpr int rows = PANEL_H;
+        const int jl = s * W + lane * K;
+        GX_CHECK(chk, i0 + rows <= ma && i0 + rows <= mb && s + 1 < (int)pa->S && s + 1 < (int)pb->S && pa->col0 == 0u && pb->col0 == 0u, 16);
+        GX_CHECK(chk, BR == 32, 16);
+
+        const uint8_t *ga = seq + pa->s1_off + i0, *gb = seq + pb->s1_off + i0;
+        const uint32_t da = (uint32_t)(reinterpret_cast<uintptr_t>(ga) & 15u), db = (uint32_t)(reinterpret_cast<uintptr_t>(gb) & 15u);
+        __syncwarp();
+        if (lane == 0) {
+            fence_proxy_async_smem();
+            const uint32_t ba = (da + (uint32_t)rows + 15u) & ~15u, bb = (db + (uint32_t)rows + 15u) & ~15u;
+            mbar_expect_tx(mbar, ba + bb);
+            tma_bulk_g2s(s1buf, ga - da, ba, mbar);
+            tma_bulk_g2s(s1buf_b, gb - db, bb, mbar);
+        }
+
+        uint32_t pra[K], prb[K];
+        {
+            const uint8_t *sa = seq + pa->s2_off + jl, *sb = seq + pb->s2_off + jl;
+#pragma unroll
+            for (int k = 0; k < K; ++k) {
+                const int ca = (int)__ldg(sa + k), cb = (int)__ldg(sb + k);
+                uint32_t wa = 0u, wb = 0u;
+#pragma unroll
+                for (int sym = 0; sym < 4; ++sym) {
+                    wa |= ((uint32_t)((ca == 8 * sym) ? ap : bp) & 0xffu) << (8 * sym);
+                    wb |= ((uint32_t)((cb == 8 * sym) ? ap : bp) & 0xffu) << (8 * sym);
+                }
+                pra[k] = wa;
+                prb[k] = wb;
+            }
+        }
+
+        uint32_t eu[K], du[K];
+        int base_a, base_b;
+        if (p == 0) {
+            base_a = base_b = h + (jl - lane * K + 1) * g + hg;
+#pragma unroll
+            for (int k = 0; k < K; ++k) {
+                const int v = h + (jl + k + 1) * g + hg;
+                eu[k] = dual_pack(v - base_a + DUAL_OFF, v - base_b + DUAL_OFF);
+                du[k] = 0u;
+            }
+        } else {
+            const uint32_t *pra_ = P.progress + pa->progress_off + s, *prb_ = P.progress + pb->progress_off + s;
+            uint32_t spins = 0, nap = 100;
+            bool dead_ = false;
+            const long long w0 = P.stats ? clock64() : 0;
+            while (ld_relaxed_u32(pra_) < (uint32_t)p || ld_relaxed_u32(prb_) < (uint32_t)p) {
+                if (spin_check(spins, abort_word)) {
+                    dead_ = true;
+                    break;
+                }
+                __nanosleep(nap);
+                nap = min(nap * 2u, 1000u);
+            }
+            (void)ld_acquire_u32(pra_);
+            (void)ld_acquire_u32(prb_);
+            if (P.stats) st_top += clock64() - w0;
+            if (dead_) return false;
+            const int2 *ta = P.top + pa->top_off + jl, *tb = P.top + pb->top_off + jl;
+            int2 va[K], vb[K];
+#pragma unroll
+            for (int k = 0; k < K; ++k) {
+                va[k] = ld_cg_int2(ta + k);
+                vb[k] = ld_cg_int2(tb + k);
+            }
+            base_a = __shfl_sync(FULL, va[0].x, 0);
+            base_b = __shfl_sync(FULL, vb[0].x, 0);
+#pragma unroll
+            for (int k = 0; k < K; ++k) {
+                eu[k] = dual_pack(va[k].x - base_a + DUAL_OFF, vb[k].x - base_b + DUAL_OFF);
+                du[k] = dual_pack(va[k].y - base_a + DUAL_OFF, vb[k].y - base_b + DUAL_OFF);
+            }
+        }
+        const bool has_left = s > 0;
+        const unsigned long long *cin_a = has_left ? P.colbuf + pa->colbuf_off + (uint64_t)(s - 1) * ma + i0 : nullptr;
+        const unsigned long long *cin_b = has_left ? P.colbuf + pb->colbuf_off + (uint64_t)(s - 1) * mb + i0 : nullptr;
+        unsigned long long *cout_a = P.colbuf + pa->colbuf_off + (uint64_t)s * ma + i0;
+        unsigned long long *cout_b = P.colbuf + pb->colbuf_off + (uint64_t)s * mb + i0;
+        auto parity_ok = [&](unsigned long long v) __attribute__((always_inline)) { return (((uint32_t)(v >> 32)) & 1u) == parity; };
+
+        bool dead_ = false;
+        uint32_t vd = __shfl_up_sync(FULL, eu[K - 1], 1);
+        if (lane == 0) {
+            int va_, vb_;
+            if (!has_left || p == 0) {
+                va_ = vb_ = (!has_left ? ((p == 0) ? 0 : h + i0 * g) : h + jl * g) + hg;
+            } else {
+                unsigned long long wa, wb;
+                uint32_t spins = 0;
+                while (!parity_ok(wa = ld_relaxed_u64(cin_a - 1)) || !parity_ok(wb = ld_relaxed_u64(cin_b - 1))) {
+                    if (spin_check(spins, abort_word)) {
+                        dead_ = true;
+                        break;
+                    }
+                    __nanosleep(100);
+                }
+                va_ = (int)(uint32_t)wa;
+                vb_ = (int)(uint32_t)wb;
+            }
+            vd = dual_pack(va_ - base_a + DUAL_OFF, vb_ - base_b + DUAL_OFF);
+        }
+        if (__any_sync(FULL, dead_)) return false;
+
+        uint32_t eo = 0u, io = 0u;
+        const uint32_t nbat = tile_batches((uint32_t)rows, 1u, (uint32_t)B);
+        unsigned long long nxa = 0, nxb = 0;
+        const bool lane_b = lane < BR;
+        auto issue = [&](uint32_t bt) __attribute__((always_inline)) {
+            const int r = (int)(BR * bt) + lane;
+            if (has_left && lane_b && r < rows) {
+                nxa = ld_relaxed_u64(cin_a + r);
+                nxb = ld_relaxed_u64(cin_b + r);
+            }
+        };
+        if (has_left && P.start_lead > 0) {
+            const int lead = min((int)P.start_lead, rows - 1);
+            uint32_t spins = 0;
+            const long long w0 = P.stats ? clock64() : 0;
+            while (!parity_ok(ld_relaxed_u64(cin_a + lead)) || !parity_ok(ld_relaxed_u64(cin_b + lead))) {
+                if (spin_check(spins, abort_word)) {
+                    dead_ = true;
+                    break;
+                }
+                __nanosleep(500);
+            }
+            if (P.stats) st_bnd += clock64() - w0;
+            if (__any_sync(FULL, dead_)) return false;
+        }
+        issue(0);
+        {
+            uint32_t tries = 0;
+            const long long w0 = P.stats ? clock64() : 0;
+            while (!mbar_try_wait(mbar, phase)) {
+                if (++tries > (1u << 24)) {
+                    atomicExch(abort_word, 1u);
+                    dead_ = true;
+                    break;
+                }
+            }
+            if (P.stats) st_s1 += clock64() - w0;
+            if (__any_sync(FULL, dead_)) return false;
+        }
+        phase ^= 1u;
+        const uint8_t *s1a = s1buf + da, *s1b = s1buf_b + db;
+        __syncwarp();
+        uint32_t sela = dual_sel(s1a[max(-lane, 0)], s1b[max(-lane, 0)]);
+
+        auto settle = [&](uint32_t b) __attribute__((always_inline)) -> bool {
+            const int rb = (int)(BR * b) + lane;
+            const bool need = has_left && lane_b && (rb < rows);
+            bool oka = !need || parity_ok(nxa), okb = !need || parity_ok(nxb);
+            if (!__all_sync(FULL, oka && okb)) {
+                uint32_t spins = 0;
+                const long long w0 = P.stats ? clock64() : 0;
+                bool lost = false;
+                do {
+                    if (__any_sync(FULL, spin_check(spins, abort_word))) {
+                        lost = true;
+                        break;
+                    }
+                    if (P.poll_nap) __nanosleep(P.poll_nap);
+                    if (!oka) nxa = ld_relaxed_u64(cin_a + rb);
+                    if (!okb) nxb = ld_relaxed_u64(cin_b + rb);
+                    oka = !need || parity_ok(nxa);
+                    okb = !need || parity_ok(nxb);
+                } while (!__all_sync(FULL, oka && okb));
+                if (P.stats) st_bnd += clock64() - w0;
+                if (lost) return false;
+            }
+            int ea, ia, eb, ib;
+            if (has_left) {
+                ea = (int)(uint32_t)nxa;
+                ia = ((int)(uint32_t)(nxa >> 32)) >> 1;
+                eb = (int)(uint32_t)nxb;
+                ib = ((int)(uint32_t)(nxb >> 32)) >> 1;
+            } else {
+                ea = eb = h + (i0 + rb + 1) * g + hg;
+                ia = ib = NEG32;
+            }
+            GX_CHECK(chk, !need || (ea - base_a + DUAL_OFF > 0 && ea - base_a + DUAL_OFF < 32768 && eb - base_b + DUAL_OFF > 0 &&
+                                    eb - base_b + DUAL_OFF < 32768), 17);
+            if (lane_b) inring[(b & 1u) * BR + lane] = make_uint2(dual_pack(ea - base_a + DUAL_OFF, eb - base_b + DUAL_OFF),
+                                                                  dual_pack(ia - base_a + DUAL_OFF, ib - base_b + DUAL_OFF));
+            return true;
+        };
+        if (!settle(0)) return false;
+        if (nbat > 1) issue(1);
+        __syncwarp();
+        if (P.stats) tl_dp0 = globaltimer_ns();
+        const uint32_t g2 = ((uint32_t)g & 0xffffu) * 0x10001u;
+        const uint32_t hg2 = (uint32_t)(hg * 0x10001);
+        auto post = [&](uint32_t bt, const uint2 *outr) __attribute__((always_inline)) -> bool {
+            const int ro = ((int)(B * bt) - 31) + lane;
+            const bool take = lane_b && ro >= 0 && ro < rows;
+            __syncwarp();
+            if (take) {
+                const uint2 w = lds_volatile_uint2(outr + lane);
+                const int ea = dual_lo(w.x) + base_a, ia = dual_lo(w.y) + base_a, eb = dual_hi(w.x) + base_b, ib = dual_hi(w.y) + base_b;
+                st_relaxed_u64(cout_a + ro, (unsigned long long)(uint32_t)ea | ((unsigned long long)(((uint32_t)ia << 1) | parity) << 32));
+                st_relaxed_u64(cout_b + ro, (unsigned long long)(uint32_t)eb | ((unsigned long long)(((uint32_t)ib << 1) | parity) << 32));
+            }
+            const uint32_t ref = __shfl_sync(FULL, eu[0], 0);
+            const int dla = dual_lo(ref), dlb = dual_hi(ref);
+            base_a += dla;
+            base_b += dlb;
+            const uint32_t nd = ((uint32_t)(-dla) & 0xffffu) | ((uint32_t)(-dlb) << 16);
+#pragma unroll
+            for (int k = 0; k < K; ++k) {
+                GX_CHECK(chk, (int)(eu[k] & 0xffffu) - dla > 0 && (int)(eu[k] >> 16) - dlb > 0 && (int)(du[k] & 0xffffu) - dla > 0 &&
+                                  (int)(du[k] >> 16) - dlb > 0, 18);
+                eu[k] = __viaddmax_s16x2(eu[k], nd, 0u);
+                du[k] = __viaddmax_s16x2(du[k], nd, 0u);
+            }
+            eo = __viaddmax_s16x2(eo, nd, 0u);
+            io = __viaddmax_s16x2(io, nd, 0u);
+            vd = __viaddmax_s16x2(vd, nd, 0u);
+            if (bt + 1 < nbat) {
+                if (!settle(bt + 1)) return false;
+                if (bt + 2 < nbat) issue(bt + 2);
+                __syncwarp();
+            }
+            return true;
+        };
+        const uint32_t nb_body = ((uint32_t)rows) / B;
+        bool ok = true;
+        for (uint32_t bt = 0; bt < nbat && ok; ++bt) {
+            uint2 *outr = outring + (bt & 1u) * BR;
+            if (bt == 0 || bt >= nb_body)
+                run_batch_dual<K, true>(eu, du, pra, prb, eo, io, vd, g2, hg2, one, s1a, s1b, inring + (bt & 1u) * BR, outr,
+                                        (int)(B * bt), rows, lane, sela, cpb, chk);
+            else
+                run_batch_dual<K, false>(eu, du, pra, prb, eo, io, vd, g2, hg2, one, s1a, s1b, inring + (bt & 1u) * BR, outr,
+                                         (int)(B * bt), rows, lane, sela, cpb, chk);
+            ok = post(bt, outr);
+        }
+        if (!ok) return false;
+
+        {
+            int2 *ta = P.top + pa->top_off + jl, *tb = P.top + pb->top_off + jl;
+#pragma unroll
+            for (int k = 0; k < K; ++k) {
+                st_cg_int2(ta + k, make_int2(dual_lo(eu[k]) + base_a, dual_lo(du[k]) + base_a));
+                st_cg_int2(tb + k, make_int2(dual_hi(eu[k]) + base_b, dual_hi(du[k]) + base_b));
+            }
+            __syncwarp();
+            if (lane == 0) {
+                st_release_u32(P.progress + pa->progress_off + s, (uint32_t)(p + 1));
+                st_release_u32(P.progress + pb->progress_off + s, (uint32_t)(p + 1));
+            }
+        }
+        return true;
+    };
     for (;;) {
         uint32_t tk = 0;
         if (P.pmax != 0u) {
@@ -262,6 +594,33 @@
         const unsigned long long tl_take = P.stats ? globaltimer_ns() : 0ull;
         unsigned long long tl_dp0 = 0ull;
         long long st_top = 0, st_bnd = 0, st_s1 = 0;
+        auto emit_stats = [&]() __attribute__((always_inline)) {
+            if (P.stats && lane == 0) {
+                atomicAdd(P.stats + 0, (unsigned long long)st_top);
+                atomicAdd(P.stats + 1, (unsigned long long)st_bnd);
+                atomicAdd(P.stats + 2, (unsigned long long)(clock64() - st_t0));
+                atomicAdd(P.stats + 3, (unsigned long long)st_s1);
+                atomicAdd(P.stats + 4, 1ull);
+                if (P.timeline) {
+                    unsigned long long *tl = P.timeline + 4ull * tk;
+                    uint32_t smid;
+                    asm volatile("mov.u32 %0, %%smid;" : "=r"(smid));
+                    tl[0] = tl_take;
+                    tl[1] = tl_dp0;
+                    tl[2] = globaltimer_ns();
+                    tl[3] = ((unsigned long long)td.pair << 48) | ((unsigned long long)td.p << 32) | ((unsigned long long)td.s << 12) | smid;
+                }
+            }
+        };
+        if constexpr (DUAL) {
+            if (td.pad_ != 0u) {
+                if (!dual_tile(td, tl_dp0, st_top, st_bnd, st_s1)) break;
+                emit_stats();
+                continue;
+            }
+        } else {
+            GX_CHECK(chk, td.pad_ == 0u, 15);
+        }
         const PairDesc *pd = P.pairs + td.pair;
         const int m = (int)pd->m, n = (int)pd->n, S = (int)pd->S;
         const int p = (int)td.p, s = (int)td.s;
@@ -588,22 +947,7 @@
             }
             if (lane == 0) P.tile_best[pd->tile_base + p * S + s] = make_int4(bv, bi, bj, 0);
         }
-        if (P.stats && lane == 0) {
-            atomicAdd(P.stats + 0, (unsigned long long)st_top);
-            atomicAdd(P.stats + 1, (unsigned long long)st_bnd);
-            atomicAdd(P.stats + 2, (unsigned long long)(clock64() - st_t0));
-            atomicAdd(P.stats + 3, (unsigned long long)st_s1);
-            atomicAdd(P.stats + 4, 1ull);
-            if (P.timeline) {
-                unsigned long long *tl = P.timeline + 4ull * tk;
-                uint32_t smid;
-                asm volatile("mov.u32 %0, %%smid;" : "=r"(smid));
-                tl[0] = tl_take;
-                tl[1] = tl_dp0;
-                tl[2] = globaltimer_ns();
-                tl[3] = ((unsigned long long)td.pair << 48) | ((unsigned long long)p << 32) | ((unsigned long long)s << 12) | smid;
-            }
-        }
+        emit_stats();
     }
 }
 
diff --git a/include/gxalign.h b/include/gxalign.h
--- a/include/gxalign.h
+++ b/include/gxalign.h
@@ -102,6 +102,9 @@
 
 int gx_debug_tile_order(const uint64_t *len1, const uint64_t *len2, uint64_t n_pairs, int K, int bands, uint32_t *out,
                         uint64_t cap_tiles, uint64_t *n_tiles);
+int gx_debug_dual_order(const uint64_t *len1, const uint64_t *len2, uint64_t n_pairs, int code_w, uint32_t *out,
+                        uint64_t cap_entries, uint64_t *n_entries);
+int gx_dual_frame_ok(gx_scores sc, int K, int batch_steps);
 
 int gx_replay_ops(const uint8_t *ops, uint64_t n_ops, uint64_t start_i, uint64_t start_j,
                   uint32_t *ops_i, uint32_t *ops_j);
```

New measurement: 3039, median of 6. +3.2%, better.
